# AdrianPerezHerrero/HDP-GPC

Measured on AMD Instinct MI355X. Metric: GP log-lik evals/sec (NxK batch, T-point segments), higher is better.
Workload: dtype f64; 1 GPU; BASELINE configs[1]: synthetic 2048 segments x 8 clusters, T=128, fp64, irregular segment grids (per-pair Gram + Cholesky + score); segments=2048, segments_per_gpu=2048, clusters=8, T=128

## Files before the change

### hdpgpc_amd/csrc/hgp_factor.hip

```cpp
#include <mutex>

#include "hgp_internal.hpp"
#include "tile_f64.hpp"

using namespace hgp;

namespace {

template <int NB>
__global__ __launch_bounds__(64 * WAVES) void k_wave_potrf(PotrfArgs a) {
  __shared__ __attribute__((aligned(16))) double scr_all[WAVES * DIAG_SCR];
  const int wave = threadIdx.x >> 6, lane = threadIdx.x & 63;
  const int g = lane >> 4, c = lane & 15;
  const int m = blockIdx.x * WAVES + wave;
  if (m >= a.b) return;
  double* scr = scr_all + wave * DIAG_SCR;
  double* A = a.A + (size_t)m * a.T * a.T;
  const int T = a.T;
  d4 U[NB * (NB + 1) / 2];
  d4 R[NB];
  load_sym_upper<NB>(U, A, T, T, lane, scr);
  if (a.add != 0.0) add_diag<NB>(U, a.add, T, lane);
  if (a.jitter_rel != 0.0) {
    double dm = diag_abs_mean<NB>(U, T, lane);
    add_diag<NB>(U, a.jitter_rel * fmax(dm, F64_EPS), T, lane);
  }
  PivotAcc pa;
  pa.init();
  wave_factor<NB, 0>(U, R, scr, nullptr, nullptr, lane, pa, A, T, T);
#pragma unroll
  for (int I = 0; I < NB; ++I)
#pragma unroll
    for (int J = I + 1; J < NB; ++J) {
      const int ln = launder(lane);
#pragma unroll
      for (int r = 0; r < 4; ++r) {
        int i = 16 * I + (ln >> 4) + 4 * r, j = 16 * J + (ln & 15);
        if (i < T && j < T) A[(size_t)i * T + j] = 0.0;
      }
    }
  if (lane == 0) {
    if (a.info) a.info[m] = pa.info;
    if (a.logdet) a.logdet[m] = pa.logdet();
  }
}

template <int NB>
__global__ __launch_bounds__(64 * WAVES) void k_wave_inv(PotrfArgs a) {
  __shared__ __attribute__((aligned(16))) double scr_all[WAVES * DIAG_SCR];
  const int wave = threadIdx.x >> 6, lane = threadIdx.x & 63;
  const int g = lane >> 4, c = lane & 15;
  const int w = blockIdx.x * WAVES + wave;
  const int m = w / NB, Jc = w % NB;
  const int T = a.T;
  if (m >= a.b || 16 * Jc >= T) return;
  double* scr = scr_all + wave * DIAG_SCR;
  const double* A = a.A + (size_t)m * T * T;
  d4 U[NB * (NB + 1) / 2];
  d4 R[NB];
  if (a.symmetric) load_upper_only<NB>(U, A, T, T, lane);
  else if constexpr (NB <= 6) load_sym_upper_burst<NB>(U, A, T, T, lane, scr);
  else load_sym_upper<NB>(U, A, T, T, lane, scr);
  {
    double sh = a.add;
    if (a.jitter_rel != 0.0) sh += a.jitter_rel * fmax(diag_abs_mean<NB>(U, T, lane, a.add), F64_EPS);
    if (sh != 0.0) add_diag<NB>(U, sh, T, lane);
  }
#pragma unroll
  for (int K = 0; K < NB; ++K)
#pragma unroll
    for (int r = 0; r < 4; ++r) R[K][r] = (K == Jc && g + 4 * r == c) ? 1.0 : 0.0;
  PivotAcc pa;
  pa.init();
  wave_factor<NB, 1>(U, R, scr, nullptr, nullptr, lane, pa, nullptr, 0, T);
  double* Z = a.Linv + (size_t)m * T * T;
#pragma unroll
  for (int K = 0; K < NB; ++K)
#pragma unroll
    for (int r = 0; r < 4; ++r) {
      const int i = 16 * K + g + 4 * r, j = 16 * Jc + c;
      if (i < T && j < T) Z[(size_t)i * T + j] = (K >= Jc) ? R[K][r] : 0.0;
    }
  if (a.inv_info && Jc == 0 && lane == 0 && a.info) a.info[m] = pa.info;
}

template <int NB>
void launch_wave_inv(const PotrfArgs& a, hipStream_t st) {
  const int waves = a.b * NB;
  hipLaunchKernelGGL(k_wave_inv<NB>, dim3((waves + WAVES - 1) / WAVES), dim3(64 * WAVES), 0, st, a);
}

struct ScoreArgs {
  const double* Y;
  int ldy;
  const double* mean;
  long mean_stride;
  const double* Sigma;
  long sigma_stride;
  int T;
  int ld_sigma;
  const int32_t* item_mat;
  const int32_t* item_mean;
  const double* item_add;
  const int32_t* item_off;
  const int32_t* item_cnt;
  int n_items;
  const int32_t* seg_ids;
  double jitter_rel;
  double* out_quad;
  double* out_logdet;
  int32_t* out_info;
};

template <int NB>
__global__ __launch_bounds__(64 * WAVES) void k_wave_score(ScoreArgs a) {
  __shared__ __attribute__((aligned(16))) double scr_all[WAVES * DIAG_SCR];
  __shared__ __attribute__((aligned(16))) double w_all[WAVES * NB * 256];
  const int wave = threadIdx.x >> 6, lane = threadIdx.x & 63;
  const int g = lane >> 4, c = lane & 15;
  const int it = blockIdx.x * WAVES + wave;
  if (it >= a.n_items) return;
  double* scr = scr_all + wave * DIAG_SCR;
  const int T = a.T;
  const int mat = a.item_mat[it];
  const double* S = a.Sigma + (size_t)mat * a.sigma_stride;
  const double* mu = a.mean ? a.mean + (size_t)(a.item_mean ? a.item_mean[it] : mat) * a.mean_stride : nullptr;
  d4 U[NB * (NB + 1) / 2];
  d4 R[NB];
  double* Wl = w_all + wave * NB * 256;
  load_sym_upper<NB>(U, S, a.ld_sigma, T, lane, scr);
  const double add = a.item_add ? a.item_add[it] : 0.0;
  if (add != 0.0) add_diag<NB>(U, add, T, lane);
  if (a.jitter_rel != 0.0) {
    double dm = diag_abs_mean<NB>(U, T, lane);
    add_diag<NB>(U, a.jitter_rel * fmax(dm, F64_EPS), T, lane);
  }
  const int off = a.item_off[it], cnt = a.item_cnt[it];
  PivotAcc pa;
  pa.init();
  double ld = 0.0;
  for (int base = 0; base < cnt; base += 16) {
    const int j = base + c;
    const bool live = j < cnt;
    const int seg = live ? (a.seg_ids ? a.seg_ids[off + j] : off + j) : 0;
    const double* yr = a.Y + (size_t)seg * a.ldy;
#pragma unroll
    for (int K = 0; K < NB; ++K)
#pragma unroll
      for (int r = 0; r < 4; ++r) {
        int i = 16 * K + g + 4 * r;
        double v = 0.0;
        if (live && i < T) v = yr[i] - (mu ? mu[i] : 0.0);
        R[K][r] = v;
      }
    if (base == 0) {
      wave_factor<NB, 1>(U, R, scr, cnt > 16 ? Wl : nullptr, nullptr, lane, pa, nullptr, 0, T);
      ld = pa.logdet();
    } else {
      wave_fwd_solve<NB>(U, Wl, R, lane);
    }
    double q = wave_colnorm2<NB>(R);
    if (live && g == 0) {
      a.out_quad[seg] = q;
      if (a.out_logdet) a.out_logdet[seg] = ld;
      if (a.out_info) a.out_info[seg] = pa.info;
    }
  }
}

struct EachArgs {
  const double* Y;
  int ldy;
  const double* mean;
  long mean_stride;
  const double* Sigma;
  long sigma_stride;
  int T, n;
  const int32_t* seg_mat;
  const int32_t* seg_mean;
  const double* seg_add;
  double jitter_rel;
  double* out_quad;
  double* out_logdet;
  int32_t* out_info;
  int symmetric;
};

template <int NB, bool SYM>
__global__ __launch_bounds__(64 * WAVES, (NB <= 6) ? 2 : 1) void k_wave_score1(EachArgs a) {
  __shared__ __attribute__((aligned(16))) double scr_all[WAVES * DIAG_SCR];
  __shared__ __attribute__((aligned(16))) double dv_all[WAVES * 16 * NB];
  const int wave = threadIdx.x >> 6, lane = threadIdx.x & 63;
  const int seg = blockIdx.x * WAVES + wave;
  if (seg >= a.n) return;
  double* scr = scr_all + wave * DIAG_SCR;
  double* dv = dv_all + wave * 16 * NB;
  const int T = a.T;
  const int mat = a.seg_mat[seg];
  const double* S = a.Sigma + (size_t)mat * a.sigma_stride;
  const double* mu = a.mean ? a.mean + (size_t)(a.seg_mean ? a.seg_mean[seg] : mat) * a.mean_stride : nullptr;
  const double* yr = a.Y + (size_t)seg * a.ldy;
  for (int i = lane; i < 16 * NB; i += 64) dv[i] = (i < T) ? yr[i] - (mu ? mu[i] : 0.0) : 0.0;
  d4 U[NB * (NB + 1) / 2];
  d4 Rnone[NB];
  if constexpr (SYM) load_upper_only<NB>(U, S, T, T, lane);
  else load_sym_upper<NB>(U, S, T, T, lane, scr);
  {
    double sh = a.seg_add ? a.seg_add[seg] : 0.0;
    if (a.jitter_rel != 0.0) sh += a.jitter_rel * fmax(diag_abs_mean<NB>(U, T, lane, sh), F64_EPS);
    if (sh != 0.0) add_diag<NB>(U, sh, T, lane);
  }
  __builtin_amdgcn_wave_barrier();
  PivotAcc pa;
  pa.init();
  const double q = wave_factor<NB, 2, (NB < 8)>(U, Rnone, scr, nullptr, dv, lane, pa, nullptr, 0, T);
  if (lane == 0) {
    a.out_quad[seg] = q;
    if (a.out_logdet) a.out_logdet[seg] = pa.logdet();
    if (a.out_info) a.out_info[seg] = pa.info;
  }
}

template <int NB>
__global__ __launch_bounds__(64 * WAVES) void k_coop_score(ScoreArgs a) {
  using C = Coop<NB>;
  extern __shared__ __attribute__((aligned(16))) double smem[];
  double* rowbuf = smem;
  double* Rbuf = rowbuf + NB * 256;
  double* Wbuf = Rbuf + NB * 256;
  double* scr = Wbuf + 256;
  double* red = scr + DIAG_SCR;
  int* redi = reinterpret_cast<int*>(red + 8);
  const int wave = __builtin_amdgcn_readfirstlane(threadIdx.x >> 6), lane = threadIdx.x & 63;
  const int g = lane >> 4, c = lane & 15;
  const int it = blockIdx.x;
  const int T = a.T;
  const int mat = a.item_mat[it];
  const double* S = a.Sigma + (size_t)mat * a.sigma_stride;
  const double* mu = a.mean ? a.mean + (size_t)(a.item_mean ? a.item_mean[it] : mat) * a.mean_stride : nullptr;
  const double add = a.item_add ? a.item_add[it] : 0.0;
  const int off = a.item_off[it], cnt = a.item_cnt[it];
  d4 U[C::NT];
  for (int base = 0; base < cnt; base += 16) {
    coop_load_sym_upper<NB>(U, S, a.ld_sigma, T, wave, lane, rowbuf + wave * DIAG_SCR);
    __syncthreads();
    {
      double sh = add;
      if (a.jitter_rel != 0.0) {
        const double dm = coop_diag_abs_mean<NB>(U, T, wave, lane, add, red);
        sh += a.jitter_rel * fmax(dm, F64_EPS);
      }
      if (sh != 0.0) coop_add_diag<NB>(U, sh, T, wave, lane);
    }
    const int j = base + c;
    const bool live = j < cnt;
    const int seg = live ? (a.seg_ids ? a.seg_ids[off + j] : off + j) : 0;
    const double* yr = a.Y + (size_t)seg * a.ldy;
    for (int K = wave; K < NB; K += WAVES) {
      d4 v;
#pragma unroll
      for (int r = 0; r < 4; ++r) {
        const int i = 16 * K + g + 4 * r;
        v[r] = (live && i < T) ? yr[i] - (mu ? mu[i] : 0.0) : 0.0;
      }
      lds_tile_store(Rbuf, K, lane, v);
    }
    __syncthreads();
    PivotAcc pa;
    pa.init();
    coop_factor<NB, true>(U, rowbuf, Rbuf, Wbuf, scr, wave, lane, pa, nullptr, 0, T);
    int info;
    const double ld = coop_logdet_info(pa, wave, lane, red, redi, info);
    double q = 0.0;
    for (int K = wave; K < NB; K += WAVES) {
      const d4 z = lds_tile_load(Rbuf, K, lane);
#pragma unroll
      for (int r = 0; r < 4; ++r) q = fma(z[r], z[r], q);
    }
    q = xrow_sum(q);
    if (g == 0) Wbuf[wave * 16 + c] = q;
    __syncthreads();
    if (wave == 0 && g == 0 && live) {
      a.out_quad[seg] = Wbuf[c] + Wbuf[16 + c] + Wbuf[32 + c] + Wbuf[48 + c];
      if (a.out_logdet) a.out_logdet[seg] = ld;
      if (a.out_info) a.out_info[seg] = info;
    }
    __syncthreads();
  }
}

template <int NB>
__global__ __launch_bounds__(64 * WAVES) void k_coop_potrf(PotrfArgs a) {
  using C = Coop<NB>;
  extern __shared__ __attribute__((aligned(16))) double smem[];
  double* rowbuf = smem;
  double* Rbuf = rowbuf + NB * 256;
  double* Wbuf = Rbuf + NB * 256;
  double* scr = Wbuf + 256;
  double* red = scr + DIAG_SCR;
  int* redi = reinterpret_cast<int*>(red + 8);
  const int wave = __builtin_amdgcn_readfirstlane(threadIdx.x >> 6), lane = threadIdx.x & 63;
  const int m = blockIdx.x;
  const int T = a.T;
  double* A = (a.Aout ? a.Aout : a.A) + (size_t)m * T * T;
  d4 U[C::NT];
  coop_load_sym_upper<NB>(U, a.A + (size_t)m * T * T, T, T, wave, lane, rowbuf + wave * DIAG_SCR);
  __syncthreads();
  {
    double sh = a.add;
    if (a.jitter_rel != 0.0) {
      const double dm = coop_diag_abs_mean<NB>(U, T, wave, lane, a.add, red);
      sh += a.jitter_rel * fmax(dm, F64_EPS);
    }
    if (sh != 0.0) coop_add_diag<NB>(U, sh, T, wave, lane);
  }
  __syncthreads();
  PivotAcc pa;
  pa.init();
  coop_factor<NB, false>(U, rowbuf, Rbuf, Wbuf, scr, wave, lane, pa, A, T, T, nullptr,
                         a.Linv ? a.Linv + (size_t)m * T * T : nullptr, T);
  int info;
  const double ld = coop_logdet_info(pa, wave, lane, red, redi, info);
  if (threadIdx.x == 0) {
    if (a.info) a.info[m] = info;
    if (a.logdet) a.logdet[m] = ld;
  }
  for (int idx = threadIdx.x; idx < T * T; idx += 64 * WAVES) {
    const int i = idx / T, j = idx % T;
    if ((j >> 4) > (i >> 4)) A[idx] = 0.0;
  }
}

template <int NB>
__global__ __launch_bounds__(64 * WAVES) void k_trtri(const double* __restrict__ Lall, double* __restrict__ Zall, int T, int b,
                                                      const int32_t* __restrict__ info) {
  const int wave = threadIdx.x >> 6, lane = threadIdx.x & 63;
  const int g = lane >> 4, c = lane & 15;
  const int w = blockIdx.x * WAVES + wave;
  const int m = w / NB, Kc = w % NB;
  if (m >= b || 16 * Kc >= T) return;
  const double* L = Lall + (size_t)m * T * T;
  double* Z = Zall + (size_t)m * T * T;
  const int nb = (T + 15) >> 4;
  d4 Zc[NB];
#pragma unroll
  for (int I = 0; I < NB; ++I) {
    if (I == Kc) {
#pragma unroll
      for (int r = 0; r < 4; ++r) {
        const int row = 16 * I + g + 4 * r, col = 16 * I + c;
        Zc[I][r] = (row < T && col < T) ? Z[(size_t)row * T + col] : ((row == col) ? 1.0 : 0.0);
      }
    } else {
      Zc[I] = (d4){0.0, 0.0, 0.0, 0.0};
    }
  }
#pragma unroll
  for (int I = 1; I < NB; ++I) {
    if (I > Kc && I < nb) {
      d4 acc0 = (d4){0.0, 0.0, 0.0, 0.0}, acc1 = (d4){0.0, 0.0, 0.0, 0.0};
#pragma unroll
      for (int j = 0; j < I; ++j) {
        if (j >= Kc) {
          double av[4];
#pragma unroll
          for (int s = 0; s < 4; ++s) {
            const int row = 16 * I + c, col = 16 * j + 4 * s + g;
            av[s] = (row < T) ? L[(size_t)row * T + col] : 0.0;
          }
          if (j & 1) {
#pragma unroll
            for (int s = 0; s < 4; ++s) acc1 = mfma(av[s], Zc[j][s], acc1);
          } else {
#pragma unroll
            for (int s = 0; s < 4; ++s) acc0 = mfma(av[s], Zc[j][s], acc0);
          }
        }
      }
#pragma unroll
      for (int r = 0; r < 4; ++r) acc0[r] += acc1[r];
      double wv[4];
#pragma unroll
      for (int s = 0; s < 4; ++s) {
        const int row = 16 * I + c, col = 16 * I + 4 * s + g;
        wv[s] = (row < T && col < T) ? Z[(size_t)row * T + col] : ((row == col) ? 1.0 : 0.0);
      }
      d4 z = (d4){0.0, 0.0, 0.0, 0.0};
#pragma unroll
      for (int s = 0; s < 4; ++s) z = mfma_sub(wv[s], acc0[s], z);
      Zc[I] = z;
    }
  }
  const bool bad = info && info[m] != 0;
#pragma unroll
  for (int I = 0; I < NB; ++I) {
#pragma unroll
    for (int r = 0; r < 4; ++r) {
      const int row = 16 * I + g + 4 * r, col = 16 * Kc + c;
      if (row < T && col < T && I != Kc) Z[(size_t)row * T + col] = bad ? __builtin_nan("") : ((I > Kc) ? Zc[I][r] : 0.0);
    }
  }
}

template <int NB>
__global__ __launch_bounds__(64 * WAVES) void k_coop_inv(PotrfArgs a) {
  using C = Coop<NB>;
  extern __shared__ __attribute__((aligned(16))) double smem[];
  double* rowbuf = smem;
  double* Rbuf = rowbuf + NB * 256;
  double* Wbuf = Rbuf + NB * 256;
  double* scr = Wbuf + 256;
  double* red = scr + DIAG_SCR;
  const int wave = __builtin_amdgcn_readfirstlane(threadIdx.x >> 6), lane = threadIdx.x & 63;
  const int g = lane >> 4, c = lane & 15;
  const int m = blockIdx.x, Jc = blockIdx.y;
  const int T = a.T;
  if (16 * Jc >= T) return;
  const double* A = a.A + (size_t)m * T * T;
  d4 U[C::NT];
  coop_load_sym_upper<NB>(U, A, T, T, wave, lane, rowbuf + wave * DIAG_SCR);
  __syncthreads();
  {
    double sh = a.add;
    if (a.jitter_rel != 0.0) {
      const double dm = coop_diag_abs_mean<NB>(U, T, wave, lane, a.add, red);
      sh += a.jitter_rel * fmax(dm, F64_EPS);
    }
    if (sh != 0.0) coop_add_diag<NB>(U, sh, T, wave, lane);
  }
  for (int K = wave; K < NB; K += WAVES) {
    d4 v;
#pragma unroll
    for (int r = 0; r < 4; ++r) v[r] = (K == Jc && g + 4 * r == c) ? 1.0 : 0.0;
    lds_tile_store(Rbuf, K, lane, v);
  }
  __syncthreads();
  PivotAcc pa;
  pa.init();
  coop_factor<NB, true>(U, rowbuf, Rbuf, Wbuf, scr, wave, lane, pa, nullptr, 0, T);
  double* Z = a.Linv + (size_t)m * T * T;
  for (int K = wave; K < NB; K += WAVES) {
    const d4 z = lds_tile_load(Rbuf, K, lane);
#pragma unroll
    for (int r = 0; r < 4; ++r) {
      const int i = 16 * K + g + 4 * r, j = 16 * Jc + c;
      if (i < T && j < T) Z[(size_t)i * T + j] = (K >= Jc) ? z[r] : 0.0;
    }
  }
  if (a.inv_info && Jc == 0) {
    int info;
    (void)coop_logdet_info(pa, wave, lane, red, reinterpret_cast<int*>(red + 8), info);
    if (threadIdx.x == 0 && a.info) a.info[m] = info;
  }
}

template <int NB>
int launch_coop_score(const ScoreArgs& a, hipStream_t st) {
  const size_t lds = sizeof(double) * Coop<NB>::LDS_DOUBLES;
  if (int rc_ = hgp_internal_ensure_dynamic_lds(reinterpret_cast<const void*>(&k_coop_score<NB>), lds)) return rc_;
  hipLaunchKernelGGL(k_coop_score<NB>, dim3(a.n_items), dim3(64 * WAVES), lds, st, a);
  return launch_status();
}

template <int NB>
int launch_coop_potrf(const PotrfArgs& a, hipStream_t st) {
  const size_t lds = sizeof(double) * Coop<NB>::LDS_DOUBLES;
  if (int rc_ = hgp_internal_ensure_dynamic_lds(reinterpret_cast<const void*>(&k_coop_potrf<NB>), lds)) return rc_;
  if (int rc_ = hgp_internal_ensure_dynamic_lds(reinterpret_cast<const void*>(&k_coop_inv<NB>), lds)) return rc_;
  hipLaunchKernelGGL(k_coop_potrf<NB>, dim3(a.b), dim3(64 * WAVES), lds, st, a);
  if (a.Linv) {
    const int waves = a.b * NB;
    hipLaunchKernelGGL(k_trtri<NB>, dim3((waves + WAVES - 1) / WAVES), dim3(64 * WAVES), 0, st, a.Aout ? a.Aout : a.A, a.Linv, a.T, a.b,
                       a.info);
  }
  return launch_status();
}

template <int NB>
int launch_coop_inv_only(const PotrfArgs& a, hipStream_t st) {
  const size_t lds = sizeof(double) * Coop<NB>::LDS_DOUBLES;
  if (int rc_ = hgp_internal_ensure_dynamic_lds(reinterpret_cast<const void*>(&k_coop_inv<NB>), lds)) return rc_;
  hipLaunchKernelGGL(k_coop_inv<NB>, dim3(a.b, NB), dim3(64 * WAVES), lds, st, a);
  return launch_status();
}

}

int hgp_internal_ensure_dynamic_lds(const void* fn, size_t bytes) {
  static std::mutex mu;
  static std::vector<std::pair<const void*, int>> done;
  int dv = 0;
  if (hipGetDevice(&dv) != hipSuccess) return launch_status();
  std::lock_guard<std::mutex> lk(mu);
  for (const auto& d : done)
    if (d.first == fn && d.second == dv) return 0;
  const hipError_t e = hipFuncSetAttribute(fn, hipFuncAttributeMaxDynamicSharedMemorySize, (int)bytes);
  if (e != hipSuccess) return 1000 + (int)e;
  done.emplace_back(fn, dv);
  return 0;
}

int hgp_internal_chol_inverse(const PotrfArgs& a, int NB, hipStream_t st) {
  if (NB > 8) return dispatch_nb_coop(16 * NB, [&](auto nb) { return launch_coop_potrf<decltype(nb)::value>(a, st); });
  if (NB == 8) return launch_coop_inv_only<8>(a, st);
  dispatch_nb_wave(16 * NB, [&](auto nb) { launch_wave_inv<decltype(nb)::value>(a, st); });
  return launch_status();
}

extern "C" {

int hgp_potrf_batched_f64(double* A, int T, int b, double jitter_rel, double add_diag, double* Linv, double* logdet,
                          int32_t* info, void* stream) {
  if (b == 0) return 0;
  if (!A || T <= 0 || b < 0) return -1;
  if (T > HGP_MAX_T_COOP) return -2;
  PotrfArgs a{A, T, b, jitter_rel, add_diag, Linv, logdet, info};
  hipStream_t st = (hipStream_t)stream;
  if (T > HGP_MAX_T_WAVE) return dispatch_nb_coop(T, [&](auto nb) { return launch_coop_potrf<decltype(nb)::value>(a, st); });
  dispatch_nb_wave(T, [&](auto nb) {
    constexpr int NB = decltype(nb)::value;
    if (Linv) launch_wave_inv<NB>(a, st);
    hipLaunchKernelGGL(k_wave_potrf<NB>, dim3((b + WAVES - 1) / WAVES), dim3(64 * WAVES), 0, st, a);
  });
  return launch_status();
}

int hgp_score_groups_f64(const double* Y, int ldy, const double* mean, long mean_stride, const double* Sigma,
                         long sigma_stride, int T, const int32_t* item_mat, const int32_t* item_mean,
                         const double* item_add, const int32_t* item_off, const int32_t* item_cnt, int n_items,
                         const int32_t* seg_ids, double jitter_rel, double* out_quad, double* out_logdet,
                         int32_t* out_info, void* stream) {
  if (n_items == 0) return 0;
  if (!Y || !Sigma || !item_mat || !item_off || !item_cnt || !out_quad || T <= 0 || ldy < T || n_items < 0) return -1;
  if (T > HGP_MAX_T_COOP) return -2;
  ScoreArgs a{Y, ldy, mean, mean_stride, Sigma, sigma_stride, T, T, item_mat, item_mean, item_add, item_off, item_cnt, n_items,
              seg_ids, jitter_rel, out_quad, out_logdet, out_info};
  hipStream_t st = (hipStream_t)stream;
  if (T > HGP_MAX_T_WAVE) return dispatch_nb_coop(T, [&](auto nb) { return launch_coop_score<decltype(nb)::value>(a, st); });
  dispatch_nb_wave(T, [&](auto nb) {
    hipLaunchKernelGGL(k_wave_score<decltype(nb)::value>, dim3((n_items + WAVES - 1) / WAVES), dim3(64 * WAVES), 0, st, a);
  });
  return launch_status();
}

int hgp_score_each_f64(const double* Y, int ldy, const double* mean, long mean_stride, const double* Sigma,
                       long sigma_stride, int T, const int32_t* seg_mat, const int32_t* seg_mean, const double* seg_add,
                       int n, double jitter_rel, int symmetric, double* out_quad, double* out_logdet, int32_t* out_info,
                       void* stream) {
  if (n == 0) return 0;
  if (!Y || !Sigma || !seg_mat || !out_quad || T <= 0 || ldy < T || n < 0) return -1;
  if (T > HGP_MAX_T_WAVE) return -2;
  EachArgs a{Y, ldy, mean, mean_stride, Sigma, sigma_stride, T, n, seg_mat, seg_mean, seg_add, jitter_rel, out_quad, out_logdet,
             out_info, symmetric};
  hipStream_t st = (hipStream_t)stream;
  dispatch_nb_wave(T, [&](auto nb) {
    dispatch_bool(symmetric != 0, [&](auto sym) {
      hipLaunchKernelGGL((k_wave_score1<decltype(nb)::value, decltype(sym)::value>), dim3((n + WAVES - 1) / WAVES), dim3(64 * WAVES), 0, st, a);
    });
  });
  return launch_status();
}

int hgp_chol_inverse_batched_f64(const double* A, int T, int b, double jitter_rel, double add_diag, double* Linv,
                                 int32_t* info, void* stream) {
  if (b == 0) return 0;
  if (!A || !Linv || T <= 0 || b < 0) return -1;
  if (T > HGP_MAX_T_COOP) return -2;
  PotrfArgs a{const_cast<double*>(A), T, b, jitter_rel, add_diag, Linv, nullptr, info};
  a.inv_info = 1;
  hipStream_t st = (hipStream_t)stream;
  if (T > HGP_MAX_T_WAVE) return dispatch_nb_coop(T, [&](auto nb) { return launch_coop_inv_only<decltype(nb)::value>(a, st); });
  dispatch_nb_wave(T, [&](auto nb) { launch_wave_inv<decltype(nb)::value>(a, st); });
  return launch_status();
}

int hgp_chol_inverse_ws_f64(const double* A, int T, int b, double jitter_rel, double add_diag, double* Linv, double* work,
                            int32_t* info, void* stream) {
  if (b == 0) return 0;
  if (!A || !Linv || T <= 0 || b < 0) return -1;
  if (T > HGP_MAX_T_COOP) return -2;
  const int nb = T <= 192 ? 12 : 16;
  if (T <= HGP_MAX_T_WAVE || !work || (long)b * nb <= 512) return hgp_chol_inverse_batched_f64(A, T, b, jitter_rel, add_diag, Linv, info, stream);
  PotrfArgs a{const_cast<double*>(A), T, b, jitter_rel, add_diag, Linv, nullptr, info};
  a.Aout = work;
  return dispatch_nb_coop(T, [&](auto nbc) { return launch_coop_potrf<decltype(nbc)::value>(a, (hipStream_t)stream); });
}

}
```

### hdpgpc_amd/csrc/hgp_gemm.hip

```cpp
#include <algorithm>

#include "hgp_internal.hpp"
#include "tile_f64.hpp"

using namespace hgp;

namespace {

template <int TRIP>
__global__ __launch_bounds__(64 * WAVES) void k_gemm(GemmArgs a) {
  const int wave = threadIdx.x >> 6, lane = threadIdx.x & 63;
  const int g = lane >> 4, c = lane & 15;
  const int ntn = (a.N + 15) / 16, ntm = (a.M + 15) / 16;
  const int tile = blockIdx.x * WAVES + wave;
  if (tile >= ntm * ntn) return;
  const int ti = tile / ntn, tj = tile % ntn;
  const int by = (int)blockIdx.y + a.boff;
  const int b1 = by / a.nb2, b2 = by % a.nb2;
  const double* A = a.A + (size_t)b1 * a.sA + (size_t)b2 * a.sA2;
  const double* B = a.B + (size_t)b1 * a.sB + (size_t)b2 * a.sB2;
  double* C = a.C + (size_t)b1 * a.sC + (size_t)b2 * a.sC2;
  d4 acc = (d4){0.0, 0.0, 0.0, 0.0};
  const int row = 16 * ti + c, col = 16 * tj + c;
  int nk = (a.Kd + 3) / 4;
  if (a.triA && !a.tA) nk = min(nk, 4 * (ti + 1));
  for (int k0 = 0; k0 < nk; k0 += TRIP) {
    double av[TRIP], bv[TRIP];
#pragma unroll
    for (int u = 0; u < TRIP; ++u) {
      const int k = 4 * (k0 + u) + g;
      av[u] = 0.0;
      bv[u] = 0.0;
      if (k < a.Kd) {
        if (row < a.M) av[u] = a.tA ? A[(size_t)k * a.lda + row] : A[(size_t)row * a.lda + k];
        if (col < a.N) bv[u] = a.tB ? B[(size_t)col * a.ldb + k] : B[(size_t)k * a.ldb + col];
      }
    }
#pragma unroll
    for (int u = 0; u < TRIP; ++u) acc = mfma(av[u], bv[u], acc);
  }
#pragma unroll
  for (int r = 0; r < 4; ++r) {
    const int i = 16 * ti + g + 4 * r;
    if (i < a.M && col < a.N) {
      double v = a.alpha * acc[r];
      if (a.beta != 0.0)
        v += a.beta * (a.D ? a.D[(size_t)b1 * a.sD + (size_t)i * a.ldd + col] : C[(size_t)i * a.ldc + col]);
      C[(size_t)i * a.ldc + col] = v;
    }
  }
}

__global__ __launch_bounds__(64 * WAVES) void k_gemm22(GemmArgs a) {
  const int wave = threadIdx.x >> 6, lane = threadIdx.x & 63;
  const int g = lane >> 4, c = lane & 15;
  const int ntn = a.N / 32, ntm = a.M / 32;
  const int tile = blockIdx.x * WAVES + wave;
  if (tile >= ntm * ntn) return;
  const int ti = tile / ntn, tj = tile % ntn;
  const int by = (int)blockIdx.y + a.boff;
  const int b1 = by / a.nb2, b2 = by % a.nb2;
  const double* A = a.A + (size_t)b1 * a.sA + (size_t)b2 * a.sA2 + (size_t)(32 * ti + c) * a.lda + g;
  const double* B = a.B + (size_t)b1 * a.sB + (size_t)b2 * a.sB2 + (size_t)g * a.ldb + 32 * tj + c;
  double* C = a.C + (size_t)b1 * a.sC + (size_t)b2 * a.sC2;
  d4 acc[2][2];
#pragma unroll
  for (int i = 0; i < 2; ++i)
#pragma unroll
    for (int j = 0; j < 2; ++j) acc[i][j] = (d4){0.0, 0.0, 0.0, 0.0};
  int nk = a.Kd / 4;
  if (a.triA) nk = min(nk, 8 * (ti + 1));
  constexpr int TR = 8;
  for (int k0 = 0; k0 < nk; k0 += TR) {
    double av[TR][2], bv[TR][2];
#pragma unroll
    for (int u = 0; u < TR; ++u) {
      const size_t k = 4 * (size_t)(k0 + u);
      av[u][0] = A[k];
      av[u][1] = A[k + 16 * (size_t)a.lda];
      bv[u][0] = B[k * a.ldb];
      bv[u][1] = B[k * a.ldb + 16];
    }
#pragma unroll
    for (int u = 0; u < TR; ++u) {
#pragma unroll
      for (int i = 0; i < 2; ++i)
#pragma unroll
        for (int j = 0; j < 2; ++j) acc[i][j] = mfma(av[u][i], bv[u][j], acc[i][j]);
    }
  }
#pragma unroll
  for (int i = 0; i < 2; ++i)
#pragma unroll
    for (int j = 0; j < 2; ++j)
#pragma unroll
      for (int r = 0; r < 4; ++r) {
        const int row = 32 * ti + 16 * i + g + 4 * r, col = 32 * tj + 16 * j + c;
        double v = a.alpha * acc[i][j][r];
        if (a.beta != 0.0) v += a.beta * (a.D ? a.D[(size_t)b1 * a.sD + (size_t)row * a.ldd + col] : C[(size_t)row * a.ldc + col]);
        C[(size_t)row * a.ldc + col] = v;
      }
}

__global__ __launch_bounds__(256) void k_dot_batched(const double* __restrict__ X, const double* __restrict__ Y, long sX,
                                                      long sY, long n, double scale, int accumulate, double* out) {
  __shared__ double red[256];
  const double* x = X + (size_t)blockIdx.x * sX;
  const double* y = Y + (size_t)blockIdx.x * sY;
  double s = 0.0;
  for (long i = threadIdx.x; i < n; i += 256) s = fma(x[i], y[i], s);
  red[threadIdx.x] = s;
  __syncthreads();
  for (int o = 128; o > 0; o >>= 1) {
    if (threadIdx.x < o) red[threadIdx.x] += red[threadIdx.x + o];
    __syncthreads();
  }
  if (threadIdx.x == 0) out[blockIdx.x] = (accumulate ? out[blockIdx.x] : 0.0) + scale * red[0];
}

__global__ __launch_bounds__(256) void k_colnorm_diag(const double* __restrict__ Z, const double* __restrict__ S, long sS, int T,
                                                       double scale, int accumulate, double* out) {
  __shared__ double red[256];
  const double* z = Z + (size_t)blockIdx.x * T * T;
  const double* sd = S + (size_t)blockIdx.x * sS;
  double s = 0.0;
  for (long i = threadIdx.x; i < (long)T * T; i += 256) {
    const int r = (int)(i / T), cidx = (int)(i % T);
    if (cidx <= r) {
      const double v = z[i];
      s = fma(v * v, sd[(size_t)cidx * T + cidx], s);
    }
  }
  red[threadIdx.x] = s;
  __syncthreads();
  for (int o = 128; o > 0; o >>= 1) {
    if (threadIdx.x < o) red[threadIdx.x] += red[threadIdx.x + o];
    __syncthreads();
  }
  if (threadIdx.x == 0) out[blockIdx.x] = (accumulate ? out[blockIdx.x] : 0.0) + scale * red[0];
}

__global__ void k_sub_batched(const double* __restrict__ A, const double* __restrict__ B, long sA, long sB, long n,
                              double* __restrict__ C, int b) {
  const size_t i = (size_t)blockIdx.x * blockDim.x + threadIdx.x;
  if (i >= (size_t)n) return;
  for (int m = blockIdx.y; m < b; m += gridDim.y) C[(size_t)m * n + i] = A[(size_t)m * sA + i] - B[(size_t)m * sB + i];
}

}

int hgp_internal_gemm(const GemmArgs& a0, int batch, hipStream_t st) {
  const int nt = ((a0.M + 15) / 16) * ((a0.N + 15) / 16);
  for (int b0 = 0; b0 < batch; b0 += 65535) {
    GemmArgs a = a0;
    a.boff = b0;
    const int nb = std::min(65535, batch - b0);
    if (!a.tA && !a.tB && a.M % 32 == 0 && a.N % 32 == 0 && a.Kd % 32 == 0 && a.Kd > 128 &&
        (long)(a.M / 32) * (a.N / 32) * nb >= 2048) {
      const int nt2 = (a.M / 32) * (a.N / 32);
      hipLaunchKernelGGL(k_gemm22, dim3((nt2 + WAVES - 1) / WAVES, nb), dim3(64 * WAVES), 0, st, a);
      continue;
    }
    if (a.Kd <= 96 && a.Kd > 32)
      hipLaunchKernelGGL(k_gemm<24>, dim3((nt + WAVES - 1) / WAVES, nb), dim3(64 * WAVES), 0, st, a);
    else if (a.Kd <= 128 && a.Kd > 96)
      hipLaunchKernelGGL(k_gemm<32>, dim3((nt + WAVES - 1) / WAVES, nb), dim3(64 * WAVES), 0, st, a);
    else
      hipLaunchKernelGGL(k_gemm<8>, dim3((nt + WAVES - 1) / WAVES, nb), dim3(64 * WAVES), 0, st, a);
  }
  return launch_status();
}

void hgp_internal_dot_batched(const double* X, const double* Y, long sX, long sY, long n, double scale, int accumulate, double* out, int b, hipStream_t st) {
  hipLaunchKernelGGL(k_dot_batched, dim3(b), dim3(256), 0, st, X, Y, sX, sY, n, scale, accumulate, out);
}

void hgp_internal_colnorm_diag(const double* Z, const double* S, long sS, int T, double scale, int accumulate, double* out, int b, hipStream_t st) {
  hipLaunchKernelGGL(k_colnorm_diag, dim3(b), dim3(256), 0, st, Z, S, sS, T, scale, accumulate, out);
}

void hgp_internal_sub_batched(const double* A, const double* B, long sA, long sB, long n, double* C, int b, hipStream_t st) {
  hipLaunchKernelGGL(k_sub_batched, dim3((unsigned)((n + 255) / 256), std::min(b, 65535)), dim3(256), 0, st, A, B, sA, sB, n, C, b);
}

extern "C" {

int hgp_gemm_batched_f64(int transA, int transB, int M, int N, int Kd, double alpha, const double* A, int lda, long strideA,
                         const double* B, int ldb, long strideB, double beta, double* C, int ldc, long strideC, int batch,
                         void* stream) {
  if (!A || !B || !C || M <= 0 || N <= 0 || Kd <= 0 || batch < 0) return -1;
  if (batch == 0) return 0;
  GemmArgs g{A, B, C, M, N, Kd, lda, ldb, ldc, strideA, strideB, strideC, alpha, beta, transA, transB};
  return hgp_internal_gemm(g, batch, (hipStream_t)stream);
}

int hgp_gemm_add_batched_f64(int transA, int transB, int M, int N, int Kd, double alpha, const double* A, int lda, long strideA,
                             const double* B, int ldb, long strideB, double beta, const double* D, int ldd, long strideD,
                             double* C, int ldc, long strideC, int batch, void* stream) {
  if (!A || !B || !C || !D || M <= 0 || N <= 0 || Kd <= 0 || batch < 0) return -1;
  if (batch == 0) return 0;
  GemmArgs g{A, B, C, M, N, Kd, lda, ldb, ldc, strideA, strideB, strideC, alpha, beta, transA, transB};
  g.D = D;
  g.ldd = ldd;
  g.sD = strideD;
  return hgp_internal_gemm(g, batch, (hipStream_t)stream);
}

}
```

### hdpgpc_amd/csrc/hgp_internal.hpp

```cpp
#pragma once
#include <hip/hip_runtime.h>
#include <stdint.h>
#include <stdlib.h>

#include <type_traits>
#include <vector>

#include "../../include/hdpgpc_hip.h"

constexpr int WAVES = 4;

static inline int launch_status() {
  hipError_t e = hipGetLastError();
  return e == hipSuccess ? 0 : 1000 + (int)e;
}

static inline int nb_for(int n) {
  int nb = (n + 15) / 16;
  nb = (nb + 1) & ~1;
  return nb < 2 ? 2 : nb;
}

template <class F> static inline auto dispatch_nb_wave(int T, F&& f) {
  switch (nb_for(T)) {
    case 2: return f(std::integral_constant<int, 2>{});
    case 4: return f(std::integral_constant<int, 4>{});
    case 6: return f(std::integral_constant<int, 6>{});
    default: return f(std::integral_constant<int, 8>{});
  }
}
template <class F> static inline auto dispatch_nb_coop(int T, F&& f) {
  return T <= 192 ? f(std::integral_constant<int, 12>{}) : f(std::integral_constant<int, 16>{});
}
template <class F> static inline auto dispatch_nb(int NB, F&& f) {
  return NB <= 8 ? dispatch_nb_wave(16 * NB, f) : dispatch_nb_coop(16 * NB, f);
}
template <class F> static inline auto dispatch_bool(bool on, F&& f) {
  return on ? f(std::true_type{}) : f(std::false_type{});
}

static inline bool env_on(const char* name) {
  const char* v = getenv(name);
  return v && v[0] && v[0] != '0';
}

constexpr double PAIRS_CUT = 55.45177444479562;
constexpr int PAIRS_FB_CAP = 65536;

static inline int acc_grid_for(int nb) { return nb > 8 ? 256 : 512; }

struct hgp_pairs_plan {
  int T, K, TP, NB;
  std::vector<double> theta;
  std::vector<int32_t> perm;
  std::vector<int> grp_beg, grp_end;
  std::vector<double> grp_ell;
  double *d_theta, *d_scal, *d_A, *d_S, *d_Z, *d_Kinv, *d_P, *d_Q, *d_Mp, *d_ap, *d_xb;
  int32_t* d_perm;
  bool coop = false;
  double* d_escr = nullptr;
  int32_t* d_eflags = nullptr;
  int nscr = 0;
  long escr_stride = 0;
  double acc_tol = 1e-9;
  double* d_Lop = nullptr;
  double* d_LTop = nullptr;
  double* d_Dop = nullptr;
  double* d_Sop = nullptr;
  double* d_mu = nullptr;
  int32_t* d_acc_list = nullptr;
  double* d_sscr = nullptr;
  int32_t* d_fb = nullptr;
  int score_out = 0;
};

struct PotrfArgs {
  double* A;
  int T, b;
  double jitter_rel, add;
  double* Linv;
  double* logdet;
  int32_t* info;
  int inv_info = 0;
  int symmetric = 0;
  double* Aout = nullptr;
};
int hgp_internal_chol_inverse(const PotrfArgs& a, int NB, hipStream_t st);
int hgp_internal_ensure_dynamic_lds(const void* fn, size_t bytes);

struct GemmArgs {
  const double* A;
  const double* B;
  double* C;
  int M, N, Kd, lda, ldb, ldc;
  long sA, sB, sC;
  double alpha, beta;
  int tA, tB;
  int nb2 = 1;
  long sA2 = 0, sB2 = 0, sC2 = 0;
  const double* D = nullptr;
  int ldd = 0;
  long sD = 0;
  int boff = 0;
  int triA = 0;
};
int hgp_internal_gemm(const GemmArgs& a, int batch, hipStream_t st);
void hgp_internal_dot_batched(const double* X, const double* Y, long sX, long sY, long n, double scale, int accumulate, double* out, int b, hipStream_t st);
void hgp_internal_colnorm_diag(const double* Z, const double* S, long sS, int T, double scale, int accumulate, double* out, int b, hipStream_t st);
void hgp_internal_sub_batched(const double* A, const double* B, long sA, long sB, long n, double* C, int b, hipStream_t st);

int hgp_internal_acc_prep(hgp_pairs_plan* p, const double* mean, hipStream_t st);
int hgp_internal_pairs_acc(const hgp_pairs_plan* p, const double* x, const double* y, int N, int Ts, const double* first_noise,
                           const int32_t* sel, double* out_quad, double* out_logdet, int32_t* out_info, hipStream_t st);
size_t hgp_internal_acc_bytes(int TP, int K, size_t* sizes );

int hgp_internal_lat_coop(const double* f_cur, const double* f_prev, const double* A, const double* Gamma, const double* P, int T, int b,
                          double* out, int32_t* info, double* ws, hipStream_t st);
int hgp_internal_mniw_coop(const double* M, const double* Sigma, const double* m_mean, const double* scale, long prior_stride, int T, int b,
                           double* out, int32_t* info, double* ws, hipStream_t st);

struct PairsArgs {
  const double* x;
  const double* y;
  int N, Ts;
  const double* xb;
  int T;
  const double* Mp;
  const double* ap;
  const double* scal;
  const int32_t* perm;
  int kbeg, kend;
  double ell;
  const double* first_noise;
  const int32_t* sel;
#ifdef HGP_STAMPS
  unsigned long long* stamps;
#endif
  int K;
  double* out_quad;
  double* out_logdet;
  int32_t* out_info;
  double* escr;
  int32_t* eflags;
  int nscr;
  long escr_stride;
  int flags;
  double score_add;
  int score_on;
  int32_t* fb;
};

#ifdef HGP_STAMPS
extern unsigned long long* hgp_internal_stamp_dev;
#endif
int hgp_internal_pairs_fast(const PairsArgs& a, int NB, bool coop, hipStream_t st);
```

### hdpgpc_amd/csrc/hgp_pairs_acc.hip

```cpp
#include <hip/hip_runtime.h>
#include <math.h>
#include <stdint.h>

#include "hgp_internal.hpp"
#include "tile_f64.hpp"

using namespace hgp;

namespace {

__host__ __device__ constexpr int ntl(int NB) { return NB * (NB - 1) / 2; }
__host__ __device__ constexpr int tl(int K, int Kp) { return K * (K - 1) / 2 + Kp; }

__global__ void k_acc_flags(double* scal, int K, double tol, int32_t* acc_list) {
  if (threadIdx.x != 0 || blockIdx.x != 0) return;
  int n = 0;
  for (int k = 0; k < K; ++k) {
    const double ck = scal[8 * k] * scal[8 * k + 6];
    const double bound = F64_EPS * ck * ck;
    const bool flag = (tol == 0.0) || (tol > 0.0 && !(bound <= tol));
    scal[8 * k + 7] = flag ? 1.0 : 0.0;
    if (flag) acc_list[1 + n++] = k;
  }
  acc_list[0] = n;
}

template <int NB>
__global__ __launch_bounds__(64) void k_acc_factor(double* A, int TP, const double* scal, int32_t* info) {
  __shared__ __attribute__((aligned(16))) double scr[DIAG_SCR];
  const int k = blockIdx.x, lane = threadIdx.x;
  if (scal[8 * k + 7] == 0.0) return;
  double* Ak = A + (size_t)k * TP * TP;
  d4 U[NB * (NB + 1) / 2];
  d4 R[NB];
  load_upper_only<NB>(U, Ak, TP, TP, lane);
  PivotAcc pa;
  pa.init();
  wave_factor<NB, 0>(U, R, scr, nullptr, nullptr, lane, pa, Ak, TP, TP);
  if (lane == 0 && info && pa.info != 0) info[k] = pa.info;
}

struct AccPrepArgs {
  const double* L;
  const double* S;
  const double* mean;
  const double* scal;
  int T, TP, NB;
  double* Lop;
  double* LTop;
  double* Dop;
  double* Sop;
  double* mu;
};

__global__ __launch_bounds__(256) void k_acc_prep(AccPrepArgs a) {
  const int k = blockIdx.x;
  if (a.scal[8 * k + 7] == 0.0) return;
  const int lane = threadIdx.x & 63, g = lane >> 4, c = lane & 15;
  const int wv = blockIdx.y * 4 + (threadIdx.x >> 6), nwv = gridDim.y * 4;
  const int NB = a.NB, TP = a.TP;
  const double* L = a.L + (size_t)k * TP * TP;
  const double* S = a.S + (size_t)k * TP * TP;
  const int nl = ntl(NB);
  double* Lop = a.Lop + (size_t)k * nl * 256;
  double* LTop = a.LTop + (size_t)k * nl * 256;
  double* Dop = a.Dop + (size_t)k * 4 * NB * 256;
  double* Sop = a.Sop + (size_t)k * NB * NB * 256;
  if (blockIdx.y == 0)
    for (int i = threadIdx.x; i < TP; i += 256) a.mu[(size_t)k * TP + i] = (i < a.T) ? a.mean[(size_t)k * a.T + i] : 0.0;
  const int items = nl + NB + NB * NB;
  for (int it = wv; it < items; it += nwv) {
    if (it < nl) {
      int Kb = 1;
      while (tl(Kb + 1, 0) <= it) ++Kb;
      const int Kp = it - tl(Kb, 0);
      d4 lo, lt;
#pragma unroll
      for (int s = 0; s < 4; ++s) {
        lo[s] = L[(size_t)(16 * Kb + c) * TP + 16 * Kp + 4 * s + g];
        lt[s] = L[(size_t)(16 * Kb + 4 * s + g) * TP + 16 * Kp + c];
      }
      *reinterpret_cast<d4*>(Lop + ((size_t)it * 64 + lane) * 4) = lo;
      *reinterpret_cast<d4*>(LTop + ((size_t)it * 64 + lane) * 4) = lt;
    } else if (it < nl + NB) {
      const int Kb = it - nl;
      const double* D = L + (size_t)(16 * Kb) * TP + 16 * Kb;
      d4 a1, a2, a1t, a2t;
#pragma unroll
      for (int r = 0; r < 4; ++r) {
        const double* B = D + (size_t)(4 * r) * TP + 4 * r;
        const double l00 = B[0], l10 = B[TP], l11 = B[TP + 1], l20 = B[2 * TP], l21 = B[2 * TP + 1], l22 = B[2 * TP + 2],
                     l30 = B[3 * (size_t)TP], l31 = B[3 * (size_t)TP + 1], l32 = B[3 * (size_t)TP + 2], l33 = B[3 * (size_t)TP + 3];
        double w[4][4];
#pragma unroll
        for (int i = 0; i < 4; ++i)
#pragma unroll
          for (int j = 0; j < 4; ++j) w[i][j] = 0.0;
        const double r0 = 1.0 / l00, r1 = 1.0 / l11, r2 = 1.0 / l22, r3 = 1.0 / l33;
        w[0][0] = r0;
        w[1][0] = -(l10 * w[0][0]) * r1;
        w[2][0] = -(l20 * w[0][0] + l21 * w[1][0]) * r2;
        w[3][0] = -(l30 * w[0][0] + l31 * w[1][0] + l32 * w[2][0]) * r3;
        w[1][1] = r1;
        w[2][1] = -(l21 * w[1][1]) * r2;
        w[3][1] = -(l31 * w[1][1] + l32 * w[2][1]) * r3;
        w[2][2] = r2;
        w[3][2] = -(l32 * w[2][2]) * r3;
        w[3][3] = r3;
        const int ci = c & 3;
        double wf = 0.0, wt = 0.0;
#pragma unroll
        for (int i = 0; i < 4; ++i)
#pragma unroll
          for (int j = 0; j < 4; ++j) {
            if (i == ci && j == g) wf = w[i][j];
            if (i == g && j == ci) wt = w[i][j];
          }
        const bool mine = (c >> 2) == r;
        a1[r] = mine ? wf : 0.0;
        a1t[r] = mine ? wt : 0.0;
        a2[r] = (c >= 4 * r + 4) ? D[(size_t)c * TP + 4 * r + g] : 0.0;
        a2t[r] = (c < 4 * r) ? D[(size_t)(4 * r + g) * TP + c] : 0.0;
      }
      *reinterpret_cast<d4*>(Dop + ((size_t)(0 * NB + Kb) * 64 + lane) * 4) = a1;
      *reinterpret_cast<d4*>(Dop + ((size_t)(1 * NB + Kb) * 64 + lane) * 4) = a2;
      *reinterpret_cast<d4*>(Dop + ((size_t)(2 * NB + Kb) * 64 + lane) * 4) = a1t;
      *reinterpret_cast<d4*>(Dop + ((size_t)(3 * NB + Kb) * 64 + lane) * 4) = a2t;
    } else {
      const int t = it - nl - NB, Kb = t / NB, Kp = t % NB;
      d4 so;
#pragma unroll
      for (int s = 0; s < 4; ++s) so[s] = S[(size_t)(16 * Kp + 4 * s + g) * TP + 16 * Kb + c];
      *reinterpret_cast<d4*>(Sop + ((size_t)t * 64 + lane) * 4) = so;
    }
  }
}

struct AccArgs {
  const double* x;
  const double* y;
  int N, Ts;
  const double* xb;
  int T;
  const double* scal;
  const double* mu;
  const double* Lop;
  const double* LTop;
  const double* Dop;
  const double* Sop;
  const int32_t* acc_list;
  const double* first_noise;
  const int32_t* sel;
  int K;
  double* out_quad;
  double* out_logdet;
  int32_t* out_info;
  double* sscr;
  double score_add;
  int score_on;
};

template <int NB>
struct AccLds {
  static constexpr int TP = 16 * NB;
  static constexpr size_t DOUBLES = (size_t)NB * 256  + 256  + 5 * TP  + DIAG_SCR + 32;
  static constexpr size_t BYTES = DOUBLES * sizeof(double) + 16 * sizeof(int);
};

__device__ __forceinline__ d4 ld4(const double* base, unsigned off) { return *reinterpret_cast<const d4*>(base + off); }

template <int NB>
__global__ __launch_bounds__(64 * CoopH<NB>::NW, (NB <= 8) ? 2 : 1) void k_pairs_acc(AccArgs a) {
  using H = CoopH<NB>;
  constexpr int NW = H::NW, TP = 16 * NB;
  extern __shared__ __attribute__((aligned(16))) double smem[];
  double* rowbuf = smem;
  double* Wbuf = rowbuf + NB * 256;
  double* dvec = Wbuf + 256;
  double* xs = dvec + TP;
  double* ys = xs + TP;
  double* xbs = ys + TP;
  double* mus = xbs + TP;
  double* scr = mus + TP;
  double* red = scr + DIAG_SCR;
  int* redi = reinterpret_cast<int*>(red + 32);
  const int tid = threadIdx.x, lane = tid & 63, g = lane >> 4, c = lane & 15;
  const int wave = __builtin_amdgcn_readfirstlane(tid >> 6);
  const int T = a.T, Ts = a.Ts;
  const int nflag = a.acc_list[0];
  if (nflag == 0) return;
  const long npairs = a.sel ? (long)a.N : (long)a.N * nflag;
  double* Ssc = a.sscr + (size_t)blockIdx.x * NB * NB * 256;

  for (long p = blockIdx.x; p < npairs; p += gridDim.x) {
    int n, kc;
    if (a.sel) {
      n = (int)p;
      kc = a.sel[n];
      if (a.scal[8 * kc + 7] == 0.0) continue;
    } else {
      n = (int)(p / nflag);
      kc = a.acc_list[1 + (int)(p % nflag)];
    }
    kc = __builtin_amdgcn_readfirstlane(kc);
    const double* sc = a.scal + 8 * kc;
    const double cc = sc[0], ell = sc[1], noise = sc[2];
    const bool iso = sc[3] != 0.0;
    const size_t oidx = a.sel ? (size_t)n : (size_t)n * a.K + kc;
    const double fn = a.first_noise ? a.first_noise[oidx] : 0.0;
    __syncthreads();
    for (int i = tid; i < TP; i += 64 * NW) {
      xs[i] = (i < Ts) ? a.x[(size_t)n * Ts + i] / ell : 1e150 * (double)(1 + i);
      ys[i] = (i < Ts) ? a.y[(size_t)n * Ts + i] : 0.0;
      xbs[i] = (i < T) ? a.xb[i] / ell : -1e150 * (double)(1 + i);
      mus[i] = a.mu[(size_t)kc * TP + i];
    }
    __syncthreads();
    const double* Lop = a.Lop + (size_t)kc * ntl(NB) * 256;
    const double* LTop = a.LTop + (size_t)kc * ntl(NB) * 256;
    const double* Dop = a.Dop + (size_t)kc * 4 * NB * 256;
    const double* Sop = a.Sop + (size_t)kc * NB * NB * 256;
    double* Sl = Ssc;

    double dsq = 0.0;
#pragma unroll
    for (int q = 0; q < 2; ++q) {
      const int J = (q == 0) ? wave : NB - 1 - wave;
      d4 X[NB];
#pragma unroll
      for (int K = 0; K < NB; ++K) {
        const unsigned l4 = (unsigned)launder(lane) * 4u;
        {
          const int ln = launder(lane);
          const double xj = xs[16 * J + (ln & 15)];
#pragma unroll
          for (int r = 0; r < 4; ++r) {
            const double u = xbs[16 * K + 4 * r + (ln >> 4)] - xj;
            X[K][r] = cc * exp(-0.5 * (u * u));
          }
        }
#pragma unroll
        for (int Kp = 0; Kp < K; ++Kp) {
          const d4 lo = ld4(Lop + tl(K, Kp) * 256, l4);
#pragma unroll
          for (int s = 0; s < 4; ++s) X[K] = mfma_sub(lo[s], X[Kp][s], X[K]);
        }
        const d4 a1 = ld4(Dop + (0 * NB + K) * 256, l4), a2 = ld4(Dop + (1 * NB + K) * 256, l4);
#pragma unroll
        for (int r = 0; r < 4; ++r) {
          d4 t = X[K];
          t[r] = 0.0;
          t = mfma(a1[r], X[K][r], t);
          X[K] = (r < 3) ? mfma_sub(a2[r], t[r], t) : t;
        }
      }
#pragma unroll
      for (int K = NB - 1; K >= 0; --K) {
        const unsigned l4 = (unsigned)launder(lane) * 4u;
#pragma unroll
        for (int Kp = NB - 1; Kp > K; --Kp) {
          const d4 lt = ld4(LTop + tl(Kp, K) * 256, l4);
#pragma unroll
          for (int s = 0; s < 4; ++s) X[K] = mfma_sub(lt[s], X[Kp][s], X[K]);
        }
        const d4 a1 = ld4(Dop + (2 * NB + K) * 256, l4), a2 = ld4(Dop + (3 * NB + K) * 256, l4);
#pragma unroll
        for (int r = 3; r >= 0; --r) {
          d4 t = X[K];
          t[r] = 0.0;
          t = mfma(a1[r], X[K][r], t);
          X[K] = (r > 0) ? mfma_sub(a2[r], t[r], t) : t;
        }
      }
      double pj = 0.0;
#pragma unroll
      for (int K = 0; K < NB; ++K) {
        const int ln = launder(lane);
        const unsigned l4 = (unsigned)ln * 4u;
#pragma unroll
        for (int r = 0; r < 4; ++r) pj = fma(X[K][r], mus[16 * K + 4 * r + (ln >> 4)], pj);
        *reinterpret_cast<d4*>(Sl + (K * NB + J) * 256 + l4) = X[K];
      }
      pj = xrow_sum(pj);
      if (g == 0) {
        const int j = 16 * J + c;
        const double d = ys[j] - pj;
        dvec[j] = d;
        dsq = fma(d, d, dsq);
      }
    }
    __syncthreads();

    if (iso) {
      dsq = wave_sum(dsq);
      if (lane == 0) red[wave] = dsq;
      __syncthreads();
      if (tid == 0) {
        const double v = sc[4] + fn;
        const double v2 = v + 1e-8 * fmax(fabs(v), F64_EPS);
        double tot_ = 0.0;
        for (int w_ = 0; w_ < NW; ++w_) tot_ += red[w_];
        a.out_quad[oidx] = a.score_on ? fma(-0.5, tot_ / v2, a.score_add) : (tot_ / v2);
        if (a.out_logdet) a.out_logdet[oidx] = (double)Ts * log(v2);
        if (a.out_info) a.out_info[oidx] = (v2 > 0.0) ? 0 : 1;
      }
      continue;
    }

    d4 U[H::NT];
#pragma unroll
    for (int q = 0; q < 2; ++q) {
      const int J = (q == 0) ? wave : NB - 1 - wave;
      const double xj = xs[16 * J + c];
#pragma unroll
      for (int I = 0; I < (q == 0 ? NW : NB); ++I) {
        const int ln = launder(lane);
        d4 kt = (d4){0.0, 0.0, 0.0, 0.0};
        if (I <= J) {
#pragma unroll
          for (int r = 0; r < 4; ++r) {
            const double u = xs[16 * I + (ln >> 4) + 4 * r] - xs[16 * J + (ln & 15)];
            kt[r] = cc * exp(-0.5 * (u * u));
          }
          if (I == J) {
#pragma unroll
            for (int r = 0; r < 4; ++r)
              if ((ln >> 4) + 4 * r == (ln & 15)) kt[r] = (16 * I + (ln & 15) < Ts) ? cc + noise : 1.0;
          }
          U[q == 0 ? H::slotA(I) : H::slotB(I)] = kt;
        }
      }
#pragma nounroll
      for (int K = 0; K < NB; ++K) {
        const unsigned l4 = (unsigned)launder(lane) * 4u;
        d4 Q;
#pragma unroll
        for (int r = 0; r < 4; ++r) {
          const double u = xbs[16 * K + 4 * r + g] - xj;
          Q[r] = -(cc * exp(-0.5 * (u * u)));
        }
#pragma unroll
        for (int Kp = 0; Kp < NB; ++Kp) {
          const d4 so = ld4(Sop + (K * NB + Kp) * 256, l4);
          const d4 sb = ld4(Sl + (Kp * NB + J) * 256, l4);
#pragma unroll
          for (int s = 0; s < 4; ++s) Q = mfma(so[s], sb[s], Q);
        }
#pragma unroll
        for (int I = 0; I < (q == 0 ? NW : NB); ++I) {
          if (I <= J) {
            const d4 sa = ld4(Sl + (K * NB + I) * 256, l4);
#pragma unroll
            for (int s = 0; s < 4; ++s)
              U[q == 0 ? H::slotA(I) : H::slotB(I)] = mfma(sa[s], Q[s], U[q == 0 ? H::slotA(I) : H::slotB(I)]);
          }
        }
      }
    }

    {
      const double sh = 1e-6 + fn;
      const double dm = cooph_diag_abs_mean<NB>(U, Ts, wave, lane, sh, red);
      cooph_add_diag<NB>(U, sh + 1e-8 * fmax(dm, F64_EPS), Ts, wave, lane);
    }
    PivotAcc pa;
    pa.init();
    double zq = cooph_factor<NB>(U, rowbuf, Wbuf, scr, wave, lane, pa, Ts, dvec);
    int info;
    const double ld = cooph_logdet_info<NB>(pa, wave, lane, red, redi, info);
    zq = wave_sum(zq);
    if (lane == 0) red[8 + wave] = zq;
    __syncthreads();
    if (tid == 0) {
      double tot_ = 0.0;
      for (int w_ = 0; w_ < NW; ++w_) tot_ += red[8 + w_];
      a.out_quad[oidx] = a.score_on ? fma(-0.5, tot_, a.score_add) : (tot_);
      if (a.out_logdet) a.out_logdet[oidx] = ld;
      if (a.out_info) a.out_info[oidx] = info;
    }
  }
}

template <int NB>
int launch_pairs_acc(const AccArgs& a, hipStream_t st) {
  const size_t lds = AccLds<NB>::BYTES;
  hipLaunchKernelGGL(k_pairs_acc<NB>, dim3(acc_grid_for(NB)), dim3(64 * CoopH<NB>::NW), lds, st, a);
  return launch_status();
}

}

size_t hgp_internal_acc_bytes(int TP, int K, size_t* sizes) {
  const int NB = TP / 16;
  size_t s[6];
  s[0] = (size_t)K * ntl(NB) * 256 * sizeof(double);
  s[1] = s[0];
  s[2] = (size_t)K * 4 * NB * 256 * sizeof(double);
  s[3] = (size_t)K * NB * NB * 256 * sizeof(double);
  s[4] = (size_t)K * TP * sizeof(double);
  s[5] = (size_t)acc_grid_for(NB) * NB * NB * 256 * sizeof(double);
  size_t tot = 0;
  for (int i = 0; i < 6; ++i) {
    if (sizes) sizes[i] = s[i];
    tot += (s[i] + 255) & ~(size_t)255;
  }
  return tot;
}

int hgp_internal_acc_prep(hgp_pairs_plan* p, const double* mean, hipStream_t st) {
  const int K = p->K, TP = p->TP, NB = p->NB;
  hipLaunchKernelGGL(k_acc_flags, dim3(1), dim3(64), 0, st, p->d_scal, K, p->acc_tol, p->d_acc_list);
  if (p->acc_tol < 0.0) return launch_status();
  if (NB <= 8)
    dispatch_nb_wave(TP, [&](auto nb) {
      hipLaunchKernelGGL(k_acc_factor<decltype(nb)::value>, dim3(K), dim3(64), 0, st, p->d_A, TP, p->d_scal, (int32_t*)nullptr);
    });
  AccPrepArgs a{p->d_A, p->d_S, mean, p->d_scal, p->T, TP, NB, p->d_Lop, p->d_LTop, p->d_Dop, p->d_Sop, p->d_mu};
  hipLaunchKernelGGL(k_acc_prep, dim3(K, 8), dim3(256), 0, st, a);
  return launch_status();
}

int hgp_internal_pairs_acc(const hgp_pairs_plan* p, const double* x, const double* y, int N, int Ts, const double* first_noise,
                           const int32_t* sel, double* out_quad, double* out_logdet, int32_t* out_info, hipStream_t st) {
  if (p->acc_tol < 0.0) return 0;
  AccArgs a{x, y, N, Ts, p->d_xb, p->T, p->d_scal, p->d_mu, p->d_Lop, p->d_LTop, p->d_Dop, p->d_Sop, p->d_acc_list,
            first_noise, sel, p->K, out_quad, out_logdet, out_info, p->d_sscr, -0.5 * (double)Ts * 1.8378770664093453, p->score_out};
  return dispatch_nb(p->NB, [&](auto nb) { return launch_pairs_acc<decltype(nb)::value>(a, st); });
}
```

### hdpgpc_amd/csrc/hgp_plan.hip

```cpp
#include <algorithm>
#include <new>

#include "hgp_internal.hpp"
#include "tile_f64.hpp"

using namespace hgp;

namespace {

struct PrepArgs {
  const double* xb;
  const double* mean;
  const double* Sigma;
  int T, TP, K;
  const double* theta;
  double* scal;
  double* A;
  double* S;
  double* xb_copy;
};

__global__ __launch_bounds__(256) void k_prep_build(PrepArgs a) {
  __shared__ double red[256];
  __shared__ int redi[256];
  const int k = blockIdx.x, tid = threadIdx.x;
  const int T = a.T, TP = a.TP;
  const double* Sg = a.Sigma + (size_t)k * T * T;
  const double c = a.theta[3 * k], ell = a.theta[3 * k + 1], noise = a.theta[3 * k + 2];
  double s_abs = 0.0, s_sgn = 0.0;
  for (int i = tid; i < T; i += 256) {
    double d = Sg[(size_t)i * T + i];
    s_abs += fabs(d);
    s_sgn += d;
  }
  red[tid] = s_abs;
  __syncthreads();
  for (int o = 128; o > 0; o >>= 1) {
    if (tid < o) red[tid] += red[tid + o];
    __syncthreads();
  }
  const double mean_abs = red[0] / T;
  __syncthreads();
  red[tid] = s_sgn;
  __syncthreads();
  for (int o = 128; o > 0; o >>= 1) {
    if (tid < o) red[tid] += red[tid + o];
    __syncthreads();
  }
  const double mS = red[0] / T;
  int bad = 0;
  for (int i = tid; i < T; i += 256) {
    double d = Sg[(size_t)i * T + i];
    if (!(fabs(d - mS) <= 1e-8 + 1e-5 * fabs(mS))) bad = 1;
  }
  redi[tid] = bad;
  __syncthreads();
  for (int o = 128; o > 0; o >>= 1) {
    if (tid < o) redi[tid] |= redi[tid + o];
    __syncthreads();
  }
  const double jit = 1e-4 * fmax(mean_abs, F64_EPS);
  if (tid == 0 && blockIdx.y == 0) {
    double* sc = a.scal + 8 * k;
    sc[0] = c;
    sc[1] = ell;
    sc[2] = noise;
    sc[3] = redi[0] ? 0.0 : 1.0;
    sc[4] = mS;
    sc[5] = jit;
    sc[6] = 0.0;
  }
  if (k == 0 && blockIdx.y == 0)
    for (int i = tid; i < TP; i += 256) a.xb_copy[i] = (i < T) ? a.xb[i] : 0.0;
  double* Ak = a.A + (size_t)k * TP * TP;
  double* Sk = a.S + (size_t)k * TP * TP;
  for (int idx = blockIdx.y * 256 + tid; idx < TP * TP; idx += gridDim.y * 256) {
    int i = idx / TP, j = idx % TP;
    double av, sv = 0.0;
    if (i < T && j < T) {
      double u = a.xb[i] / ell - a.xb[j] / ell;
      av = c * exp(-0.5 * (u * u));
      if (i == j) av += jit;
      sv = 0.5 * (Sg[(size_t)i * T + j] + Sg[(size_t)j * T + i]);
    } else {
      av = (i == j) ? 1.0 : 0.0;
    }
    Ak[idx] = av;
    Sk[idx] = sv;
  }
}

struct PrepFinalArgs {
  const double* Q;
  const double* Kinv;
  const double* mean;
  double* scal;
  int T, TP;
  double* Mp;
  double* ap;
  int interleave;
  int32_t* fb;
};

__global__ __launch_bounds__(256) void k_prep_final(PrepFinalArgs a) {
  const int k = blockIdx.x, tid = threadIdx.x;
  if (a.fb && k == 0 && blockIdx.y == 0 && tid == 0) {
    a.fb[0] = 0;
    a.fb[1 + PAIRS_FB_CAP] = 0;
  }
  const int T = a.T, TP = a.TP;
  const double c = a.scal[8 * k];
  const double* Q = a.Q + (size_t)k * TP * TP;
  const double* Ki = a.Kinv + (size_t)k * TP * TP;
  double* Mp = a.Mp + (size_t)k * TP * TP;
  __shared__ double tq[32][33], tk[32][33];
  const int NHh = (TP / 16) / 2, nt = TP / 32;
  const int tx = tid & 31, ty = tid >> 5;
  for (int t = blockIdx.y; t < nt * nt; t += gridDim.y) {
    const int bi = t / nt, bj = t % nt;
    __syncthreads();
#pragma unroll
    for (int r = 0; r < 4; ++r) {
      const int y = ty + 8 * r;
      tq[y][tx] = Q[(size_t)(32 * bj + y) * TP + 32 * bi + tx];
      tk[y][tx] = Ki[(size_t)(32 * bj + y) * TP + 32 * bi + tx];
    }
    __syncthreads();
#pragma unroll
    for (int r = 0; r < 4; ++r) {
      const int y = ty + 8 * r;
      const int i = 32 * bi + y, j = 32 * bj + tx;
      double v = 0.0;
      if (i < T && j < T)
        v = (c * c) * (0.5 * (Q[(size_t)i * TP + j] + tq[tx][y]) - 0.5 * (Ki[(size_t)i * TP + j] + tk[tx][y]));
      int jp = j;
      if (a.interleave) {
        const int hh = j / (16 * NHh), tl = (j / 16) % NHh, cc = j % 16;
        const int loc = (tl < 2 * (NHh / 2)) ? 32 * (tl / 2) + 2 * cc + (tl & 1) : 16 * (NHh - 1) + cc;
        jp = 16 * NHh * hh + loc;
      }
      Mp[(size_t)i * TP + jp] = v;
    }
  }
  const double* mu = a.mean + (size_t)k * T;
  __shared__ double red[256];
  double rmax = 0.0;
  for (int i = blockIdx.y * 256 + tid; i < TP; i += gridDim.y * 256) {
    double s = 0.0, rs = 0.0;
    if (i < T) {
#pragma unroll 8
      for (int j = 0; j < T; ++j) {
        const double kij = Ki[(size_t)j * TP + i];
        s = fma(kij, mu[j], s);
        rs += fabs(kij);
      }
    }
    a.ap[(size_t)k * TP + i] = c * s;
    rmax = fmax(rmax, rs);
  }
  red[tid] = rmax;
  __syncthreads();
  for (int o = 128; o > 0; o >>= 1) {
    if (tid < o) red[tid] = fmax(red[tid], red[tid + o]);
    __syncthreads();
  }
  if (tid == 0) atomicMax(reinterpret_cast<unsigned long long*>(a.scal + 8 * k + 6), (unsigned long long)__double_as_longlong(red[0]));
}

static int tp_for(int n) {
  if (n <= HGP_MAX_T_WAVE) return 16 * nb_for(n);
  return n <= 192 ? 192 : 256;
}

size_t plan_layout(hgp_pairs_plan* p, int T, int Ts_max, int K, char* base) {
  const size_t TP = (size_t)tp_for(std::max(T, Ts_max));
  const size_t mat = (size_t)K * TP * TP * sizeof(double);
  p->TP = (int)TP;
  p->NB = p->TP / 16;
  p->coop = p->TP > HGP_MAX_T_WAVE;
  size_t o = 0;
  auto take = [&](auto*& member, size_t bytes) {
    if (base) member = reinterpret_cast<std::remove_reference_t<decltype(member)>>(base + o);
    o += (bytes + 255) & ~(size_t)255;
  };
  take(p->d_theta, (size_t)K * 3 * sizeof(double));
  take(p->d_scal, (size_t)K * 8 * sizeof(double));
  take(p->d_A, mat);
  take(p->d_S, mat);
  take(p->d_Z, mat);
  take(p->d_Kinv, mat);
  take(p->d_P, mat);
  take(p->d_Q, mat);
  take(p->d_Mp, mat);
  take(p->d_ap, (size_t)K * TP * sizeof(double));
  take(p->d_perm, (size_t)K * sizeof(int32_t));
  take(p->d_xb, TP * sizeof(double));
  if (p->coop) {
    const size_t nb = (size_t)p->NB;
    const size_t cap = (nb >= 12) ? 48 : (nb == 8 ? 24 : 16);
    const size_t over = nb * nb > cap ? nb * nb - cap : 0;
    p->nscr = over ? (nb >= 12 ? 512 : 1024) : 0;
    p->escr_stride = (long)(over * 256);
    take(p->d_escr, (size_t)p->nscr * over * 256 * sizeof(double));
    take(p->d_eflags, ((size_t)p->nscr + 1) * sizeof(int32_t));
  }
  size_t sz[6];
  hgp_internal_acc_bytes((int)TP, K, sz);
  take(p->d_Lop, sz[0]);
  take(p->d_LTop, sz[1]);
  take(p->d_Dop, sz[2]);
  take(p->d_Sop, sz[3]);
  take(p->d_mu, sz[4]);
  take(p->d_sscr, sz[5]);
  take(p->d_acc_list, (size_t)(K + 1) * sizeof(int32_t));
  take(p->d_fb, (size_t)(PAIRS_FB_CAP + 2) * sizeof(int32_t));
  return o;
}

}

#ifdef HGP_STAMPS
unsigned long long* hgp_internal_stamp_dev = nullptr;
#endif

extern "C" {

size_t hgp_pairs_plan_device_bytes(int T, int Ts_max, int K) {
  if (T <= 0 || Ts_max <= 0 || K <= 0) return 0;
  hgp_pairs_plan sizing;
  return plan_layout(&sizing, T, Ts_max, K, nullptr);
}

int hgp_pairs_plan_create(hgp_pairs_plan** plan, int T, int Ts_max, int K, const double* theta_host, void* dev_buf,
                          size_t dev_bytes) {
  if (!plan || !theta_host || !dev_buf || T <= 0 || Ts_max <= 0 || K <= 0) return -1;
  if (T > HGP_MAX_T_COOP || Ts_max > HGP_MAX_T_COOP) return -2;
  if (dev_bytes < hgp_pairs_plan_device_bytes(T, Ts_max, K)) return -1;
  for (int k = 0; k < K; ++k)
    if (!(theta_host[3 * k] > 0.0) || !(theta_host[3 * k + 1] > 0.0)) return -1;
  hgp_pairs_plan* p = new (std::nothrow) hgp_pairs_plan();
  if (!p) return -1;
  p->T = T;
  p->K = K;
  p->theta.assign(theta_host, theta_host + 3 * (size_t)K);
  p->perm.resize(K);
  for (int k = 0; k < K; ++k) p->perm[k] = k;
  std::stable_sort(p->perm.begin(), p->perm.end(),
                   [&](int a, int b) { return p->theta[3 * a + 1] < p->theta[3 * b + 1]; });
  for (int i = 0; i < K;) {
    int j = i;
    double ell = p->theta[3 * p->perm[i] + 1];
    while (j < K && p->theta[3 * p->perm[j] + 1] == ell) ++j;
    p->grp_beg.push_back(i);
    p->grp_end.push_back(j);
    p->grp_ell.push_back(ell);
    i = j;
  }
  plan_layout(p, T, Ts_max, K, (char*)dev_buf);
  if (hipMemset(p->d_fb, 0, (size_t)(PAIRS_FB_CAP + 2) * sizeof(int32_t)) != hipSuccess) {
    delete p;
    return 1000 + (int)hipGetLastError();
  }
  if (p->coop && hipMemset(p->d_eflags, 0, (p->nscr + 1) * sizeof(int32_t)) != hipSuccess) {
    delete p;
    return 1000 + (int)hipGetLastError();
  }
  if (hipMemcpy(p->d_theta, p->theta.data(), sizeof(double) * 3 * K, hipMemcpyHostToDevice) != hipSuccess ||
      hipMemcpy(p->d_perm, p->perm.data(), sizeof(int32_t) * K, hipMemcpyHostToDevice) != hipSuccess) {
    delete p;
    return 1000 + (int)hipGetLastError();
  }
  *plan = p;
  return 0;
}

void hgp_pairs_plan_destroy(hgp_pairs_plan* plan) { delete plan; }

const double* hgp_pairs_plan_scalars(const hgp_pairs_plan* plan) { return plan ? plan->d_scal : nullptr; }

int hgp_pairs_plan_update(hgp_pairs_plan* p, const double* x_basis, const double* mean, const double* Sigma,
                          int32_t* info, void* stream) {
  if (!p || !x_basis || !mean || !Sigma) return -1;
  hipStream_t st = (hipStream_t)stream;
  const int K = p->K, T = p->T, TP = p->TP;
  PrepArgs pa{x_basis, mean, Sigma, T, TP, K, p->d_theta, p->d_scal, p->d_A, p->d_S, p->d_xb};
  hipLaunchKernelGGL(k_prep_build, dim3(K, 8), dim3(256), 0, st, pa);
  PotrfArgs fa{p->d_A, TP, K, 0.0, 0.0, p->d_Z, nullptr, info};
  fa.inv_info = 1;
  fa.symmetric = 1;
  if (int rc = hgp_internal_chol_inverse(fa, p->NB, st)) return rc;
  const long sm = (long)TP * TP;
  GemmArgs g1{p->d_Z, p->d_Z, p->d_Kinv, TP, TP, TP, TP, TP, TP, sm, sm, sm, 1.0, 0.0, 1, 0};
  GemmArgs g2{p->d_S, p->d_Kinv, p->d_P, TP, TP, TP, TP, TP, TP, sm, sm, sm, 1.0, 0.0, 0, 0};
  GemmArgs g3{p->d_Kinv, p->d_P, p->d_Q, TP, TP, TP, TP, TP, TP, sm, sm, sm, 1.0, 0.0, 0, 0};
  hgp_internal_gemm(g1, K, st);
  hgp_internal_gemm(g2, K, st);
  hgp_internal_gemm(g3, K, st);
  PrepFinalArgs fin{p->d_Q, p->d_Kinv, mean, p->d_scal, T, TP, p->d_Mp, p->d_ap, p->coop ? 0 : 1, p->d_fb};
  hipLaunchKernelGGL(k_prep_final, dim3(K, 8), dim3(256), 0, st, fin);
  if (p->d_eflags && p->nscr > 0 && hipMemsetAsync(p->d_eflags, 0, (p->nscr + 1) * sizeof(int32_t), st) != hipSuccess) return launch_status();
  int rc = hgp_internal_acc_prep(p, mean, st);
  return rc ? rc : launch_status();
}

int hgp_pairs_plan_set_accuracy(hgp_pairs_plan* p, double tol) {
  if (!p || tol != tol) return -1;
  p->acc_tol = tol;
  return 0;
}

int hgp_pairs_plan_set_score_output(hgp_pairs_plan* p, int on) {
  if (!p) return -1;
  p->score_out = on ? 1 : 0;
  return 0;
}

int hgp_loglik_pairs_f64(const hgp_pairs_plan* p, const double* x, const double* y, int N, int Ts,
                         const double* first_noise, const int32_t* sel, double* out_quad, double* out_logdet,
                         int32_t* out_info, void* stream) {
  if (N == 0) return 0;
  if (!p || !x || !y || !out_quad || N < 0 || Ts <= 0) return -1;
  if (Ts > HGP_MAX_T_COOP) return -2;
  if (Ts > p->TP) return -2;
  hipStream_t st = (hipStream_t)stream;
  int rc = 0;
  if (p->coop && p->d_eflags && p->nscr > 0 &&
      hipMemsetAsync(p->d_eflags, 0, (p->nscr + 1) * sizeof(int32_t), st) != hipSuccess)
    return launch_status();
  for (size_t gi = 0; gi < p->grp_beg.size() && rc == 0; ++gi) {
    PairsArgs a{x, y, N, Ts, p->d_xb, p->T, p->d_Mp, p->d_ap, p->d_scal, p->d_perm, p->grp_beg[gi], p->grp_end[gi],
                p->grp_ell[gi], first_noise, sel,
#ifdef HGP_STAMPS
                hgp_internal_stamp_dev,
#endif
                p->K, out_quad, out_logdet, out_info, p->d_escr, p->d_eflags, p->nscr, p->escr_stride,
                env_on("HGP_PAIRS_GENERIC") ? 1 : 0, -0.5 * (double)Ts * 1.8378770664093453, p->score_out, p->d_fb};
    rc = hgp_internal_pairs_fast(a, p->NB, p->coop, st);
  }
  if (rc == 0) rc = hgp_internal_pairs_acc(p, x, y, N, Ts, first_noise, sel, out_quad, out_logdet, out_info, st);
  return rc;
}

#ifdef HGP_STAMPS
int hgp_debug_stamps(unsigned long long* out8_host) {
  if (!hgp_internal_stamp_dev) {
    if (hipMalloc(&hgp_internal_stamp_dev, 128) != hipSuccess) return 1;
    (void)hipMemset(hgp_internal_stamp_dev, 0, 128);
  }
  if (hipMemcpy(out8_host, hgp_internal_stamp_dev, 128, hipMemcpyDeviceToHost) != hipSuccess) return 1;
  (void)hipMemset(hgp_internal_stamp_dev, 0, 128);
  return 0;
}
#endif

}
```

### hdpgpc_amd/csrc/tile_f64.hpp

```cpp
#pragma once
#include <hip/hip_runtime.h>
#include <stdint.h>

#include <type_traits>

#ifdef HGP_STAMPS
#define HGP_STAMP_DECL unsigned long long hgp_t_, hgp_acc_[12] = {0, 0, 0, 0, 0, 0, 0, 0, 0, 0, 0, 0};
#define HGP_T0() hgp_t_ = __builtin_readcyclecounter()
#define HGP_ACC(i) do { unsigned long long n_ = __builtin_readcyclecounter(); hgp_acc_[i] += n_ - hgp_t_; hgp_t_ = n_; } while (0)
#else
#define HGP_STAMP_DECL
#define HGP_T0()
#define HGP_ACC(i)
#endif

namespace hgp {

typedef double d4 __attribute__((ext_vector_type(4)));
typedef double d2 __attribute__((ext_vector_type(2)));

constexpr int DIAG_LD = 18;
constexpr int DIAG_SCR = 16 * DIAG_LD;
constexpr double F64_EPS = 2.220446049250313e-16;

__host__ __device__ constexpr int tix(int I, int J, int NB) { return I * NB - (I * (I - 1)) / 2 + (J - I); }
#ifdef HGP_RACE_STRESS
__device__ __forceinline__ void hgp_sync_stress() {
  __syncthreads();
  const unsigned w = threadIdx.x >> 6;
  const unsigned h = ((w + 1u) * 2654435761u) ^ (unsigned)(__builtin_readcyclecounter() >> 9);
  const unsigned n = __builtin_amdgcn_readfirstlane(((h >> 3) & 3u) * 4u);
  for (unsigned i = 0; i < n; ++i) __builtin_amdgcn_s_sleep(32);
}
#define __syncthreads() ::hgp::hgp_sync_stress()
#endif

__host__ __device__ constexpr int ntiles(int NB) { return NB * (NB + 1) / 2; }

__device__ __forceinline__ d4 mfma(double a, double b, d4 c) {
  return __builtin_amdgcn_mfma_f64_16x16x4f64(a, b, c, 0, 0, 0);
}
__device__ __forceinline__ d4 mfma_sub(double a, double b, d4 c) {
  return __builtin_amdgcn_mfma_f64_16x16x4f64(a, b, c, 0, 0, 1);
}

__device__ __forceinline__ int launder(int x) {
  asm volatile("" : "+v"(x));
  return x;
}

__device__ __forceinline__ double launder_f64(double x) {
  asm volatile("" : "+v"(x));
  return x;
}

template <int B, int E, class F>
__device__ __forceinline__ void static_for(F&& f) {
  if constexpr (B < E) {
    f(std::integral_constant<int, B>{});
    static_for<B + 1, E>(f);
  }
}

template <int CTRL>
__device__ __forceinline__ double dpp_f64(double v) {
  const int lo = __builtin_amdgcn_mov_dpp(__double2loint(v), CTRL, 0xf, 0xf, false);
  const int hi = __builtin_amdgcn_mov_dpp(__double2hiint(v), CTRL, 0xf, 0xf, false);
  return __hiloint2double(hi, lo);
}
template <bool MAX>
__device__ __forceinline__ double wave_allreduce(double v) {
  auto op = [](double a, double b) { return MAX ? fmax(a, b) : a + b; };
  v = op(v, dpp_f64<0x128>(v));
  v = op(v, dpp_f64<0x124>(v));
  v = op(v, dpp_f64<0x122>(v));
  v = op(v, dpp_f64<0x121>(v));
  unsigned lo = (unsigned)__double2loint(v), hi = (unsigned)__double2hiint(v);
  auto a = __builtin_amdgcn_permlane16_swap(lo, lo, false, false);
  auto b = __builtin_amdgcn_permlane16_swap(hi, hi, false, false);
  v = op(__hiloint2double((int)b[0], (int)a[0]), __hiloint2double((int)b[1], (int)a[1]));
  lo = (unsigned)__double2loint(v);
  hi = (unsigned)__double2hiint(v);
  a = __builtin_amdgcn_permlane32_swap(lo, lo, false, false);
  b = __builtin_amdgcn_permlane32_swap(hi, hi, false, false);
  return op(__hiloint2double((int)b[0], (int)a[0]), __hiloint2double((int)b[1], (int)a[1]));
}

__device__ __forceinline__ double wave_sum(double v) { return wave_allreduce<false>(v); }

__device__ __forceinline__ double xrow_sum(double v) {
  unsigned lo = (unsigned)__double2loint(v), hi = (unsigned)__double2hiint(v);
  auto a = __builtin_amdgcn_permlane16_swap(lo, lo, false, false);
  auto b = __builtin_amdgcn_permlane16_swap(hi, hi, false, false);
  double s = __hiloint2double((int)b[0], (int)a[0]) + __hiloint2double((int)b[1], (int)a[1]);
  lo = (unsigned)__double2loint(s);
  hi = (unsigned)__double2hiint(s);
  a = __builtin_amdgcn_permlane32_swap(lo, lo, false, false);
  b = __builtin_amdgcn_permlane32_swap(hi, hi, false, false);
  return __hiloint2double((int)b[0], (int)a[0]) + __hiloint2double((int)b[1], (int)a[1]);
}

__device__ __forceinline__ double rsqrt_nr(double a) {
  const double y = __builtin_amdgcn_rsq(a);
  const double e = fma(-(0.5 * a * y), y, 0.5);
  return fma(y * e, fma(1.5, e, 1.0), y);
}

__device__ __forceinline__ void exp_neg4(const double (&h)[4], double (&o)[4]) {
  double n[4], r[4], p[4];
#pragma unroll
  for (int i = 0; i < 4; ++i) {
    const double t = -fmin(h[i], 800.0);
    n[i] = __builtin_rint(t * 1.4426950408889634);
    r[i] = fma(n[i], -6.93147180369123816490e-01, t);
  }
#pragma unroll
  for (int i = 0; i < 4; ++i) {
    r[i] = fma(n[i], -1.90821492927058770002e-10, r[i]);
    p[i] = 1.6059043836821613e-10;
  }
  constexpr double ck[13] = {1.0, 1.0, 0.5, 1.6666666666666666e-01, 4.1666666666666664e-02, 8.3333333333333332e-03,
                             1.3888888888888889e-03, 1.9841269841269841e-04, 2.4801587301587302e-05, 2.7557319223985893e-06,
                             2.7557319223985888e-07, 2.5052108385441720e-08, 2.0876756987868100e-09};
#pragma unroll
  for (int k = 12; k >= 0; --k) {
#pragma unroll
    for (int i = 0; i < 4; ++i) p[i] = fma(p[i], r[i], ck[k]);
  }
#pragma unroll
  for (int i = 0; i < 4; ++i) o[i] = __builtin_amdgcn_ldexp(p[i], (int)n[i]);
}

struct PivotAcc {
  double mant;
  int ex;
  int info;
#ifdef HGP_STAMPS
  unsigned long long diag_cycles, cf[5];
  __device__ __forceinline__ void init() { mant = 1.0; ex = 0; info = 0; diag_cycles = 0; for (int i = 0; i < 5; ++i) cf[i] = 0; }
#else
  __device__ __forceinline__ void init() { mant = 1.0; ex = 0; info = 0; }
#endif
  __device__ __forceinline__ void renorm() {
    ex += __builtin_amdgcn_frexp_exp(mant);
    mant = __builtin_amdgcn_frexp_mant(mant);
  }
  __device__ __forceinline__ double logdet() const { return log(mant) + (double)ex * 0.6931471805599453; }
};

__device__ __forceinline__ double lane_bcast(double v, int src) {
  int lo = __builtin_amdgcn_readlane(__double2loint(v), src);
  int hi = __builtin_amdgcn_readlane(__double2hiint(v), src);
  return __hiloint2double(hi, lo);
}

__device__ __forceinline__ double rcp_nr(double a) {
  const double y = __builtin_amdgcn_rcp(a);
  const double e = fma(-a, y, 1.0);
  const double ye = y * e;
  return fma(ye, e, y + ye);
}

__device__ __forceinline__ double row16_prod(double v) {
  v *= dpp_f64<0x128>(v);
  v *= dpp_f64<0x124>(v);
  v *= dpp_f64<0x122>(v);
  v *= dpp_f64<0x121>(v);
  return v;
}
__device__ __forceinline__ int row16_sum_i32(int v) {
  v += __builtin_amdgcn_mov_dpp(v, 0x128, 0xf, 0xf, false);
  v += __builtin_amdgcn_mov_dpp(v, 0x124, 0xf, 0xf, false);
  v += __builtin_amdgcn_mov_dpp(v, 0x122, 0xf, 0xf, false);
  v += __builtin_amdgcn_mov_dpp(v, 0x121, 0xf, 0xf, false);
  return v;
}

template <int G0>
__device__ __forceinline__ double row_to_all(double v) {
  const unsigned lo = (unsigned)__double2loint(v), hi = (unsigned)__double2hiint(v);
  const auto a = __builtin_amdgcn_permlane16_swap(lo, lo, false, false);
  const auto b = __builtin_amdgcn_permlane16_swap(hi, hi, false, false);
  const unsigned lo1 = a[G0 & 1], hi1 = b[G0 & 1];
  const auto a2 = __builtin_amdgcn_permlane32_swap(lo1, lo1, false, false);
  const auto b2 = __builtin_amdgcn_permlane32_swap(hi1, hi1, false, false);
  return __hiloint2double((int)b2[G0 >> 1], (int)a2[G0 >> 1]);
}
__device__ __forceinline__ double row_to_all_bperm(double v, int addr) {
  const int lo = __builtin_amdgcn_ds_bpermute(addr, __double2loint(v));
  const int hi = __builtin_amdgcn_ds_bpermute(addr, __double2hiint(v));
  return __hiloint2double(hi, lo);
}
template <int RS, int RMF>
__device__ __forceinline__ void elim_crit(double (&S)[4], double (&Z)[4], double mrot, double nt, double ntz) {
  asm("s_nop 1\n\t"
      "v_fmac_f64_dpp %0, %2, %3 row_newbcast:%5 row_mask:%6 bank_mask:0xf\n\t"
      "v_fmac_f64_dpp %1, %2, %4 row_newbcast:%5 row_mask:%6 bank_mask:0xf"
      : "+v"(S[RS]), "+v"(Z[RS])
      : "v"(mrot), "v"(nt), "v"(ntz), "n"(4 * RS), "n"(RMF));
}
template <int RS>
__device__ __forceinline__ void elim_rest(double (&S)[4], double (&Z)[4], double mrot, double nt, double ntz) {
#define HGP_FD(dst, mul, lane) "v_fmac_f64_dpp %" #dst ", %6, %" #mul " row_newbcast:" #lane " row_mask:0xf bank_mask:0xf\n\t"
  if constexpr (RS == 0) {
    asm("s_nop 1\n\t" HGP_FD(0, 7, 4) HGP_FD(1, 7, 8) HGP_FD(2, 7, 12) HGP_FD(3, 8, 4) HGP_FD(4, 8, 8) HGP_FD(5, 8, 12)
        : "+v"(S[1]), "+v"(S[2]), "+v"(S[3]), "+v"(Z[1]), "+v"(Z[2]), "+v"(Z[3])
        : "v"(mrot), "v"(nt), "v"(ntz));
  } else if constexpr (RS == 1) {
    asm("s_nop 1\n\t" HGP_FD(1, 7, 8) HGP_FD(2, 7, 12) HGP_FD(4, 8, 8) HGP_FD(5, 8, 12)
        : "+v"(S[1]), "+v"(S[2]), "+v"(S[3]), "+v"(Z[1]), "+v"(Z[2]), "+v"(Z[3])
        : "v"(mrot), "v"(nt), "v"(ntz));
  } else if constexpr (RS == 2) {
    asm("s_nop 1\n\t" HGP_FD(2, 7, 12) HGP_FD(5, 8, 12)
        : "+v"(S[1]), "+v"(S[2]), "+v"(S[3]), "+v"(Z[1]), "+v"(Z[2]), "+v"(Z[3])
        : "v"(mrot), "v"(nt), "v"(ntz));
  }
#undef HGP_FD
}

struct NoBg {
  template <class KC>
  __device__ __forceinline__ void operator()(KC) const {}
};
template <class BG = NoBg>
__device__ __forceinline__ d4 diag16_acc(const d4& X, double* scr, int lane, PivotAcc& pa, int col0,
                                         double* Lout, int ldl, int nvalid, BG&& bg = BG{}) {
  const int g = lane >> 4, c = lane & 15;
#ifdef HGP_STAMPS
  const unsigned long long td0 = __builtin_readcyclecounter();
#endif
  double S[4], Z[4];
  d4 Us;
#pragma unroll
  for (int r = 0; r < 4; ++r) {
    S[r] = X[r];
    Z[r] = (4 * r + g == c) ? 1.0 : 0.0;
    Us[r] = 0.0;
  }
  int pvlo = 0, pvhi = 0;
  const int crot = (c + g) & 15;
  double p = lane_bcast(S[0], 0);
  double sk = row_to_all_bperm(S[0], 4 * c), mrot = row_to_all_bperm(S[0], 4 * crot), zk = row_to_all_bperm(Z[0], 4 * c);
  static_for<0, 15>([&](auto kc) {
    constexpr int k = decltype(kc)::value, r0 = k >> 2, g0 = k & 3;
    constexpr int RS = (g0 == 3) ? r0 + 1 : r0;
    constexpr int RMF = (g0 == 3) ? 0xf : (0xf << (g0 + 1)) & 0xf;
    asm("v_writelane_b32 %0, %1, %2" : "+v"(pvlo) : "s"(__double2loint(p)), "n"(k));
    asm("v_writelane_b32 %0, %1, %2" : "+v"(pvhi) : "s"(__double2hiint(p)), "n"(k));
    const double rp = rcp_nr(p);
    if (Lout != nullptr) Us[r0] = (g == g0) ? sk : Us[r0];
    const double nt = -(sk * rp), ntz = -(zk * rp), mr = mrot;
    elim_crit<RS, RMF>(S, Z, mr, nt, ntz);
    constexpr int k1 = k + 1, g1 = k1 & 3;
    p = lane_bcast(S[RS], 16 * g1 + k1);
    if constexpr (k1 < 15) {
      scr[lane] = S[RS];
      scr[64 + lane] = Z[RS];
      __builtin_amdgcn_wave_barrier();
      sk = scr[16 * g1 + c];
      zk = scr[64 + 16 * g1 + c];
      mrot = scr[16 * g1 + crot];
      __builtin_amdgcn_wave_barrier();
    }
    bg(kc);
    elim_rest<RS>(S, Z, mr, nt, ntz);
  });
  asm("v_writelane_b32 %0, %1, %2" : "+v"(pvlo) : "s"(__double2loint(p)), "n"(15));
  asm("v_writelane_b32 %0, %1, %2" : "+v"(pvhi) : "s"(__double2hiint(p)), "n"(15));
  if (Lout != nullptr) Us[3] = (g == 3) ? S[3] : Us[3];
  const double pv = row_to_all<0>(__hiloint2double(pvhi, pvlo));
  const double rc = rsqrt_nr(pv);
  {
    const unsigned long long bad = __ballot(!(pv > 0.0)) & 0xffffull;
    if (bad != 0 && pa.info == 0) pa.info = col0 + __ffsll((long long)bad);
    pa.mant *= row16_prod(__builtin_amdgcn_frexp_mant(pv));
    pa.ex += row16_sum_i32(__builtin_amdgcn_frexp_exp(pv));
    pa.renorm();
  }
  if (Lout != nullptr) {
#pragma unroll
    for (int r = 0; r < 4; ++r) scr[(4 * r + g) * DIAG_LD + c] = Us[r];
    if (g == 0) scr[c * DIAG_LD + 16] = rc;
    __builtin_amdgcn_wave_barrier();
    if (lane < 16 && lane < nvalid) {
#pragma unroll
      for (int i = 0; i < 16; ++i)
        if (i < nvalid) Lout[(size_t)lane * ldl + i] = (i <= lane) ? scr[i * DIAG_LD + lane] * scr[i * DIAG_LD + 16] : 0.0;
    }
    __builtin_amdgcn_wave_barrier();
  }
#pragma unroll
  for (int r = 0; r < 4; ++r) scr[(4 * r + g) * DIAG_LD + c] = Z[r];
  __builtin_amdgcn_wave_barrier();
  d4 w;
#pragma unroll
  for (int s = 0; s < 4; ++s) w[s] = scr[c * DIAG_LD + 4 * s + g] * rc;
  __builtin_amdgcn_wave_barrier();
#ifdef HGP_STAMPS
  asm volatile("s_waitcnt lgkmcnt(0)" ::: "memory");
  pa.diag_cycles += __builtin_readcyclecounter() - td0;
#endif
  return w;
}

template <int NB, int Kp>
struct Pending {
  static constexpr int M = NB - 1 - Kp, NT = M * (M + 1) / 2 - 1, N = 4 * NT, CH = (N + 14) / 15;
  static constexpr int row(int t) {
    int u = t + 1, I = Kp + 1;
    while (u >= NB - I) { u -= NB - I; ++I; }
    return I;
  }
  static constexpr int col(int t) {
    int u = t + 1, I = Kp + 1;
    while (u >= NB - I) { u -= NB - I; ++I; }
    return I + u;
  }
};
template <int NB, int RHSMODE, bool RHS_DEFER = false>
__device__ __forceinline__ double wave_factor(d4 (&U)[NB * (NB + 1) / 2], d4 (&R)[NB], double* scr, double* Wlds,
                                              double* dvec, int lane_in, PivotAcc& pa, double* Lout, int ldl, int n) {
  constexpr bool RHS = (RHSMODE == 1);
  double zq = 0.0;
  double dp[NB];
#pragma unroll
  for (int K = 0; K < NB; ++K) dp[K] = 0.0;
  static_for<0, NB>([&](auto Kc) {
    constexpr int K = decltype(Kc)::value;
    const int lane = launder(lane_in);
    const int g = lane >> 4, c = lane & 15;
    double* Ld = (Lout != nullptr) ? Lout + (size_t)(16 * K) * ldl + 16 * K : nullptr;
    d4 W;
    if constexpr (K > 0 && K + 1 < NB) {
      using P = Pending<NB, K - 1>;
      W = diag16_acc(U[tix(K, K, NB)], scr, lane, pa, 16 * K, Ld, ldl, n - 16 * K, [&](auto kc) {
        constexpr int k = decltype(kc)::value, q0 = k * P::CH, q1 = (q0 + P::CH < P::N) ? q0 + P::CH : P::N;
        static_for<q0, q1>([&](auto qc) {
          constexpr int q = decltype(qc)::value, s = q / P::NT, t = q % P::NT, I = P::row(t), J = P::col(t);
          U[tix(I, J, NB)] = mfma_sub(U[tix(K - 1, I, NB)][s], U[tix(K - 1, J, NB)][s], U[tix(I, J, NB)]);
        });
      });
    } else {
      W = diag16_acc(U[tix(K, K, NB)], scr, lane, pa, 16 * K, Ld, ldl, n - 16 * K);
    }
    if (Wlds != nullptr) {
#pragma unroll
      for (int s = 0; s < 4; ++s) Wlds[(K * 4 + s) * 64 + lane] = W[s];
    }
    if (RHSMODE == 2) {
      if (RHS_DEFER && K > 0) {
        const double q = xrow_sum(dp[K]);
        if (g == 0) dvec[16 * K + c] -= q;
        __builtin_amdgcn_wave_barrier();
      }
      double p = 0.0;
#pragma unroll
      for (int s = 0; s < 4; ++s) p = fma(W[s], dvec[16 * K + 4 * s + g], p);
      p = xrow_sum(p);
      __builtin_amdgcn_wave_barrier();
      if (g == 0) {
        dvec[16 * K + c] = p;
        zq = fma(p, p, zq);
      }
      __builtin_amdgcn_wave_barrier();
    }
#pragma unroll
    for (int J0 = K + 1; J0 <= NB; J0 += 2) {
      d4 acc0 = (d4){0.0, 0.0, 0.0, 0.0}, acc1 = (d4){0.0, 0.0, 0.0, 0.0};
      const int J1 = J0 + 1;
      const bool has0 = (J0 < NB) || RHS, has1 = (J1 < NB) || (RHS && J1 == NB);
#pragma unroll
      for (int s = 0; s < 4; ++s) {
        if (has0) acc0 = mfma(W[s], (J0 < NB) ? U[tix(K, J0 < NB ? J0 : K, NB)][s] : R[K][s], acc0);
        if (has1) acc1 = mfma(W[s], (J1 < NB) ? U[tix(K, J1 < NB ? J1 : K, NB)][s] : R[K][s], acc1);
      }
      if (J0 < NB) U[tix(K, J0 < NB ? J0 : K, NB)] = acc0;
      else if (RHS) R[K] = acc0;
      if (J1 < NB) U[tix(K, J1 < NB ? J1 : K, NB)] = acc1;
      else if (RHS && J1 == NB) R[K] = acc1;
    }
    if (Lout != nullptr) {
#pragma unroll
      for (int J = K + 1; J < NB; ++J) {
#pragma unroll
        for (int r = 0; r < 4; ++r) {
          int row = 16 * J + c, col = 16 * K + g + 4 * r;
          if (row < n && col < n) Lout[(size_t)row * ldl + col] = U[tix(K, J, NB)][r];
        }
      }
    }
    if (RHSMODE == 2 && K + 1 < NB) {
      double zr[4];
#pragma unroll
      for (int r = 0; r < 4; ++r) zr[r] = dvec[16 * K + g + 4 * r];
      if (RHS_DEFER) {
#pragma unroll
        for (int I = K + 1; I < NB; ++I) {
#pragma unroll
          for (int r = 0; r < 4; ++r) dp[I] = fma(U[tix(K, I, NB)][r], zr[r], dp[I]);
        }
      } else {
#pragma unroll
        for (int I = K + 1; I < NB; ++I) {
          double q = 0.0;
#pragma unroll
          for (int r = 0; r < 4; ++r) q = fma(U[tix(K, I, NB)][r], zr[r], q);
          q = xrow_sum(q);
          if (g == 0) dvec[16 * I + c] -= q;
        }
        __builtin_amdgcn_wave_barrier();
      }
    }
#pragma unroll
    for (int I = K + 1; I < NB; ++I) {
#pragma unroll
      for (int s = 0; s < 4; ++s) {
#pragma unroll
        for (int J = I; J < NB; ++J) {
          if (K + 2 < NB && !(I == K + 1 && J == K + 1)) continue;
          U[tix(I, J, NB)] = mfma_sub(U[tix(K, I, NB)][s], U[tix(K, J, NB)][s], U[tix(I, J, NB)]);
        }
        if (RHS) R[I] = mfma_sub(U[tix(K, I, NB)][s], R[K][s], R[I]);
      }
    }
  });
  return (RHSMODE == 2) ? wave_sum(zq) : 0.0;
}

template <int NB>
__device__ __forceinline__ void wave_fwd_solve(const d4 (&U)[NB * (NB + 1) / 2], const double* Wlds, d4 (&R)[NB],
                                               int lane, int K0 = 0) {
#pragma unroll
  for (int K = 0; K < NB; ++K) {
    if (K < K0) continue;
    d4 t = R[K];
#pragma unroll
    for (int I = 0; I < K; ++I) {
      if (I < K0) continue;
#pragma unroll
      for (int s = 0; s < 4; ++s) t = mfma_sub(U[tix(I, K, NB)][s], R[I][s], t);
    }
    d4 z = (d4){0.0, 0.0, 0.0, 0.0};
#pragma unroll
    for (int s = 0; s < 4; ++s) z = mfma(Wlds[(K * 4 + s) * 64 + lane], t[s], z);
    R[K] = z;
  }
}

template <int NB>
__device__ __forceinline__ double wave_colnorm2(const d4 (&Z)[NB]) {
  double s = 0.0;
#pragma unroll
  for (int K = 0; K < NB; ++K)
#pragma unroll
    for (int r = 0; r < 4; ++r) s = fma(Z[K][r], Z[K][r], s);
  s += __shfl_xor(s, 16, 64);
  s += __shfl_xor(s, 32, 64);
  return s;
}

template <int NB>
__device__ __forceinline__ void load_sym_upper(d4 (&U)[NB * (NB + 1) / 2], const double* __restrict__ A, int ld, int n,
                                               int lane_in, double* scr) {
#pragma unroll
  for (int I = 0; I < NB; ++I) {
    const int lane = launder(lane_in);
    const int g = lane >> 4, c = lane & 15;
    d4 nat[NB], trn[NB];
#pragma unroll
    for (int J = I; J < NB; ++J) {
#pragma unroll
      for (int r = 0; r < 4; ++r) {
        const int i = 16 * I + g + 4 * r, j = 16 * J + c;
        nat[J][r] = (i < n && j < n) ? A[(size_t)i * ld + j] : 0.0;
        const int i2 = 16 * J + g + 4 * r, j2 = 16 * I + c;
        trn[J][r] = (J > I && i2 < n && j2 < n) ? A[(size_t)i2 * ld + j2] : 0.0;
      }
    }
#pragma unroll
    for (int J = I; J < NB; ++J) {
      const d4 src = (J == I) ? nat[I] : trn[J];
#pragma unroll
      for (int r = 0; r < 4; ++r) scr[(g + 4 * r) * DIAG_LD + c] = src[r];
      __builtin_amdgcn_wave_barrier();
      d4 v;
#pragma unroll
      for (int r = 0; r < 4; ++r) {
        const int i = 16 * I + g + 4 * r, j = 16 * J + c;
        const double t = scr[c * DIAG_LD + g + 4 * r];
        double x = 0.5 * (nat[J][r] + t);
        if (!(i < n && j < n)) x = (i == j) ? 1.0 : 0.0;
        v[r] = x;
      }
      __builtin_amdgcn_wave_barrier();
      U[tix(I, J, NB)] = v;
    }
  }
}

template <int NB>
__device__ __forceinline__ void load_sym_upper_burst(d4 (&U)[NB * (NB + 1) / 2], const double* __restrict__ A, int ld, int n,
                                                     int lane_in, double* scr) {
  constexpr int NO = NB > 1 ? NB * (NB - 1) / 2 : 1;
  d4 trn[NO];
  {
    const int lane = launder(lane_in);
    const int g = lane >> 4, c = lane & 15;
#pragma unroll
    for (int I = 0; I < NB; ++I)
#pragma unroll
      for (int J = I; J < NB; ++J)
#pragma unroll
        for (int r = 0; r < 4; ++r) {
          const int i = 16 * I + g + 4 * r, j = 16 * J + c;
          U[tix(I, J, NB)][r] = (i < n && j < n) ? A[(size_t)i * ld + j] : 0.0;
          if (J > I) {
            const int i2 = 16 * J + g + 4 * r, j2 = 16 * I + c;
            trn[tix(I, J, NB) - (I + 1)][r] = (i2 < n && j2 < n) ? A[(size_t)i2 * ld + j2] : 0.0;
          }
        }
  }
#pragma unroll
  for (int I = 0; I < NB; ++I) {
#pragma unroll
    for (int J = I; J < NB; ++J) {
      const int lane = launder(lane_in);
      const int g = lane >> 4, c = lane & 15;
      const d4 nat = U[tix(I, J, NB)];
      const d4 src = (J == I) ? nat : trn[(J == I) ? 0 : tix(I, J, NB) - (I + 1)];
#pragma unroll
      for (int r = 0; r < 4; ++r) scr[(g + 4 * r) * DIAG_LD + c] = src[r];
      __builtin_amdgcn_wave_barrier();
      d4 v;
#pragma unroll
      for (int r = 0; r < 4; ++r) {
        const int i = 16 * I + g + 4 * r, j = 16 * J + c;
        const double t = scr[c * DIAG_LD + g + 4 * r];
        double x = 0.5 * (nat[r] + t);
        if (!(i < n && j < n)) x = (i == j) ? 1.0 : 0.0;
        v[r] = x;
      }
      __builtin_amdgcn_wave_barrier();
      U[tix(I, J, NB)] = v;
    }
  }
}

template <int NB>
__device__ __forceinline__ void load_upper_only(d4 (&U)[NB * (NB + 1) / 2], const double* __restrict__ A, int ld, int n,
                                                int lane_in) {
#pragma unroll
  for (int I = 0; I < NB; ++I) {
#pragma unroll
    for (int J = I; J < NB; ++J) {
      const int lane = launder(lane_in);
      const int g = lane >> 4, c = lane & 15;
      d4 v;
#pragma unroll
      for (int r = 0; r < 4; ++r) {
        int i = 16 * I + g + 4 * r, j = 16 * J + c;
        double x = 0.0;
        if (i < n && j < n) x = A[(size_t)i * ld + j];
        else if (i == j) x = 1.0;
        v[r] = x;
      }
      U[tix(I, J, NB)] = v;
    }
  }
}

template <int NB>
__device__ __forceinline__ void add_diag(d4 (&U)[NB * (NB + 1) / 2], double shift, int n, int lane_in) {
#pragma unroll
  for (int I = 0; I < NB; ++I) {
    const int lane = launder(lane_in);
    const int g = lane >> 4, c = lane & 15;
#pragma unroll
    for (int r = 0; r < 4; ++r) {
      int i = 16 * I + g + 4 * r;
      if (g + 4 * r == c && i < n) U[tix(I, I, NB)][r] += shift;
    }
  }
}

template <int NB>
__device__ __forceinline__ double diag_abs_mean(const d4 (&U)[NB * (NB + 1) / 2], int n, int lane_in, double shift = 0.0) {
  double s = 0.0;
#pragma unroll
  for (int I = 0; I < NB; ++I) {
    const int lane = launder(lane_in);
    const int g = lane >> 4, c = lane & 15;
#pragma unroll
    for (int r = 0; r < 4; ++r) {
      int i = 16 * I + g + 4 * r;
      if (g + 4 * r == c && i < n) s += fabs(U[tix(I, I, NB)][r] + shift);
    }
  }
  return wave_sum(s) / (double)n;
}

template <int NB>
struct Coop {
  static_assert(NB % 4 == 0 && NB <= 16, "cooperative factor: NB in {4,8,12,16}");
  static constexpr int NQ = NB / 4;
  static constexpr int NT = 2 * NQ * (NQ + 1);
  __host__ __device__ static constexpr int loc(int I, int q) { return 2 * q * (q + 1) + I; }
  __host__ __device__ static constexpr int col(int q, int wave) { return 4 * q + ((q & 1) ? 3 - wave : wave); }
  __host__ __device__ static constexpr int owner(int J) { return ((J >> 2) & 1) ? 3 - (J & 3) : (J & 3); }
  static constexpr int LDS_DOUBLES = NB * 256  + NB * 256  + 256  + DIAG_SCR + 16;
};

__device__ __forceinline__ d4 lds_tile_load(const double* buf, int tile, int lane) {
  d4 v;
#pragma unroll
  for (int r = 0; r < 4; ++r) v[r] = buf[(tile * 4 + r) * 64 + lane];
  return v;
}
__device__ __forceinline__ void lds_tile_store(double* buf, int tile, int lane, const d4& v) {
#pragma unroll
  for (int r = 0; r < 4; ++r) buf[(tile * 4 + r) * 64 + lane] = v[r];
}

template <int NB>
__device__ __forceinline__ void coop_load_sym_upper(d4 (&U)[Coop<NB>::NT], const double* __restrict__ A, int ld, int n,
                                                    int wave, int lane_in, double* scr_w) {
#pragma unroll
  for (int q = 0; q < Coop<NB>::NQ; ++q) {
    const int lane = launder(lane_in);
    const int g = lane >> 4, c = lane & 15;
    const int J = Coop<NB>::col(q, wave);
    d4 nat[NB], trn[NB];
#pragma unroll
    for (int I = 0; I < 4 * q + 4; ++I) {
#pragma unroll
      for (int r = 0; r < 4; ++r) {
        const int i = 16 * I + g + 4 * r, j = 16 * J + c;
        nat[I][r] = (I <= J && i < n && j < n) ? A[(size_t)i * ld + j] : 0.0;
        const int i2 = 16 * J + g + 4 * r, j2 = 16 * I + c;
        trn[I][r] = (I < J && i2 < n && j2 < n) ? A[(size_t)i2 * ld + j2] : 0.0;
      }
    }
#pragma unroll
    for (int I = 0; I < 4 * q + 4; ++I) {
      const d4 src = (I == J) ? nat[I] : trn[I];
#pragma unroll
      for (int r = 0; r < 4; ++r) scr_w[(g + 4 * r) * DIAG_LD + c] = src[r];
      __builtin_amdgcn_wave_barrier();
      d4 v = (d4){0.0, 0.0, 0.0, 0.0};
#pragma unroll
      for (int r = 0; r < 4; ++r) {
        const int i = 16 * I + g + 4 * r, j = 16 * J + c;
        const double t = scr_w[c * DIAG_LD + g + 4 * r];
        double x = 0.5 * (nat[I][r] + t);
        if (!(i < n && j < n)) x = (i == j) ? 1.0 : 0.0;
        if (I <= J) v[r] = x;
      }
      __builtin_amdgcn_wave_barrier();
      U[Coop<NB>::loc(I, q)] = v;
    }
  }
}

template <int NB>
__device__ __forceinline__ double coop_diag_abs_mean(const d4 (&U)[Coop<NB>::NT], int n, int wave, int lane_in, double shift,
                                                     double* red) {
  double s = 0.0;
#pragma unroll
  for (int q = 0; q < Coop<NB>::NQ; ++q) {
#pragma unroll
    for (int I = 4 * q; I < 4 * q + 4; ++I) {
      const int lane = launder(lane_in);
      const int g = lane >> 4, c = lane & 15;
      if (I == Coop<NB>::col(q, wave)) {
#pragma unroll
        for (int r = 0; r < 4; ++r) {
          const int i = 16 * I + g + 4 * r;
          if (g + 4 * r == c && i < n) s += fabs(U[Coop<NB>::loc(I, q)][r] + shift);
        }
      }
    }
  }
  s = wave_sum(s);
  if (lane_in == 0) red[wave] = s;
  __syncthreads();
  const double tot = red[0] + red[1] + red[2] + red[3];
  __syncthreads();
  return tot / (double)n;
}

template <int NB>
__device__ __forceinline__ void coop_add_diag(d4 (&U)[Coop<NB>::NT], double shift, int n, int wave, int lane_in) {
#pragma unroll
  for (int q = 0; q < Coop<NB>::NQ; ++q) {
#pragma unroll
    for (int I = 4 * q; I < 4 * q + 4; ++I) {
      const int lane = launder(lane_in);
      const int g = lane >> 4, c = lane & 15;
      if (I == Coop<NB>::col(q, wave)) {
#pragma unroll
        for (int r = 0; r < 4; ++r) {
          const int i = 16 * I + g + 4 * r;
          if (g + 4 * r == c && i < n) U[Coop<NB>::loc(I, q)][r] += shift;
        }
      }
    }
  }
}

template <int NB, int RHSMODE>
__device__ __forceinline__ double coop_factor(d4 (&U)[Coop<NB>::NT], double* rowbuf, double* Rbuf, double* Wbuf, double* scr,
                                              int wave, int lane_in, PivotAcc& pa, double* Lout, int ldl, int n,
                                              double* dvec = nullptr, double* Wout = nullptr, int ldw = 0,
                                              double* Lpack = nullptr, double* Wpack = nullptr, int kstop = NB) {
  using C = Coop<NB>;
  constexpr bool RHS = (RHSMODE == 1);
  double zq = 0.0;
#ifdef HGP_STAMPS
  unsigned long long cf_t = __builtin_readcyclecounter();
#define HGP_CF(i) do { unsigned long long n_ = __builtin_readcyclecounter(); pa.cf[i] += n_ - cf_t; cf_t = n_; } while (0)
#else
#define HGP_CF(i)
#endif
#pragma unroll
  for (int K = 0; K < NB; ++K) {
    if (K >= kstop) break;
    const int qK = K / 4, wK = C::owner(K);
    const int lane = launder(lane_in);
    const int g = lane >> 4, c = lane & 15;
    if (wave == wK) {
      double* Ld = (Lout != nullptr) ? Lout + (size_t)(16 * K) * ldl + 16 * K : nullptr;
      const d4 Wd = diag16_acc(U[C::loc(K, qK)], scr, lane, pa, 16 * K, Ld, ldl, n - 16 * K);
#pragma unroll
      for (int s = 0; s < 4; ++s) Wbuf[s * 64 + lane] = Wd[s];
      if (Wout != nullptr) {
#pragma unroll
        for (int s = 0; s < 4; ++s) {
          const int row = 16 * K + c, col = 16 * K + 4 * s + g;
          if (row < n && col < n) Wout[(size_t)row * ldw + col] = Wd[s];
        }
      }
      if (Wpack != nullptr) *reinterpret_cast<d4*>(Wpack + ((size_t)K * 64 + lane) * 4) = Wd;
      if (RHS) {
        const d4 rk = lds_tile_load(Rbuf, K, lane);
        d4 z = (d4){0.0, 0.0, 0.0, 0.0};
#pragma unroll
        for (int s = 0; s < 4; ++s) z = mfma(Wd[s], rk[s], z);
        lds_tile_store(Rbuf, K, lane, z);
      }
      if (RHSMODE == 2) {
        double p = 0.0;
#pragma unroll
        for (int s = 0; s < 4; ++s) p = fma(Wd[s], dvec[16 * K + 4 * s + g], p);
        p = xrow_sum(p);
        __builtin_amdgcn_wave_barrier();
        if (g == 0) {
          dvec[16 * K + c] = p;
          zq = fma(p, p, zq);
        }
      }
    }
    HGP_CF(0);
    __syncthreads();
    HGP_CF(1);
    d4 W;
#pragma unroll
    for (int s = 0; s < 4; ++s) W[s] = Wbuf[s * 64 + lane];
#pragma unroll
    for (int q = qK; q < C::NQ; ++q) {
      const int J = Coop<NB>::col(q, wave);
      if (J > K && J < NB) {
        const d4 t = U[C::loc(K, q)];
        d4 acc = (d4){0.0, 0.0, 0.0, 0.0};
#pragma unroll
        for (int s = 0; s < 4; ++s) acc = mfma(W[s], t[s], acc);
        U[C::loc(K, q)] = acc;
        lds_tile_store(rowbuf, J, lane, acc);
        if (Lout != nullptr) {
#pragma unroll
          for (int r = 0; r < 4; ++r) {
            const int row = 16 * J + c, col = 16 * K + g + 4 * r;
            if (row < n && col < n) Lout[(size_t)row * ldl + col] = acc[r];
          }
        }
        if (Lpack != nullptr) *reinterpret_cast<d4*>(Lpack + ((size_t)(J * (J - 1) / 2 + K) * 64 + lane) * 4) = acc;
      }
    }
    if (RHSMODE == 2) {
      double zr[4];
#pragma unroll
      for (int r = 0; r < 4; ++r) zr[r] = dvec[16 * K + g + 4 * r];
#pragma unroll
      for (int q = qK; q < C::NQ; ++q) {
        const int J = Coop<NB>::col(q, wave);
        if (J > K && J < NB) {
          double t = 0.0;
#pragma unroll
          for (int r = 0; r < 4; ++r) t = fma(U[C::loc(K, q)][r], zr[r], t);
          t = xrow_sum(t);
          if (g == 0) dvec[16 * J + c] -= t;
        }
      }
    }
    HGP_CF(2);
    __syncthreads();
    HGP_CF(3);
    if (K + 1 < NB) {
      d4 ucur = lds_tile_load(rowbuf, K + 1, lane);
#pragma unroll
      for (int I = K + 1; I < NB; ++I) {
        d4 unext = ucur;
        if (I + 1 < NB) unext = lds_tile_load(rowbuf, I + 1, lane);
#pragma unroll
        for (int q = I / 4; q < C::NQ; ++q) {
          if (C::col(q, wave) >= I) {
#pragma unroll
            for (int s = 0; s < 4; ++s) U[C::loc(I, q)] = mfma_sub(ucur[s], U[C::loc(K, q)][s], U[C::loc(I, q)]);
          }
        }
        ucur = unext;
      }
    }
    if (RHS) {
      const d4 zk = lds_tile_load(Rbuf, K, lane);
#pragma unroll
      for (int I = K + 1; I < NB; ++I) {
        if (C::owner(I) == wave) {
          const d4 uki = lds_tile_load(rowbuf, I, lane);
          d4 ri = lds_tile_load(Rbuf, I, lane);
#pragma unroll
          for (int s = 0; s < 4; ++s) ri = mfma_sub(uki[s], zk[s], ri);
          lds_tile_store(Rbuf, I, lane, ri);
        }
      }
    }
    HGP_CF(4);
  }
  __syncthreads();
  return zq;
}
#undef HGP_CF

__device__ __forceinline__ double coop_logdet_info(const PivotAcc& pa, int wave, int lane, double* red, int* redi, int& info) {
  if (lane == 0) {
    red[wave] = pa.logdet();
    redi[wave] = pa.info;
  }
  __syncthreads();
  const double ld = red[0] + red[1] + red[2] + red[3];
  int inf = 0;
#pragma unroll
  for (int w = 0; w < 4; ++w)
    if (redi[w] != 0 && (inf == 0 || redi[w] < inf)) inf = redi[w];
  info = inf;
  __syncthreads();
  return ld;
}

template <int NB_>
struct CoopH {
  static_assert(NB_ % 2 == 0 && NB_ <= 16, "CoopH: even NB <= 16");
  static constexpr int NB = NB_, NT = NB_ + 1, NW = NB_ / 2;
  __host__ __device__ static constexpr int slotA(int I) { return NB - I; }
  __host__ __device__ static constexpr int slotB(int I) { return I; }
  __host__ __device__ static constexpr int owner(int J) { return J < NW ? J : NB - 1 - J; }
  __host__ __device__ static constexpr int diag_slot(int K) { return K < NW ? slotA(K) : slotB(K); }
};

template <int NB>
__device__ __forceinline__ double cooph_diag_abs_mean(const d4 (&U)[CoopH<NB>::NT], int n, int wave, int lane_in, double shift,
                                                      double* red) {
  double s = 0.0;
#pragma unroll
  for (int K = 0; K < NB; ++K) {
    const int lane = launder(lane_in);
    const int g = lane >> 4, c = lane & 15;
    if (wave == CoopH<NB>::owner(K)) {
#pragma unroll
      for (int r = 0; r < 4; ++r) {
        const int i = 16 * K + g + 4 * r;
        if (g + 4 * r == c && i < n) s += fabs(U[CoopH<NB>::diag_slot(K)][r] + shift);
      }
    }
  }
  s = wave_sum(s);
  if (lane_in == 0) red[wave] = s;
  __syncthreads();
  double tot = 0.0;
#pragma unroll
  for (int w = 0; w < CoopH<NB>::NW; ++w) tot += red[w];
  __syncthreads();
  return tot / (double)n;
}

template <int NB>
__device__ __forceinline__ void cooph_add_diag(d4 (&U)[CoopH<NB>::NT], double shift, int n, int wave, int lane_in) {
#pragma unroll
  for (int K = 0; K < NB; ++K) {
    const int lane = launder(lane_in);
    const int g = lane >> 4, c = lane & 15;
    if (wave == CoopH<NB>::owner(K)) {
#pragma unroll
      for (int r = 0; r < 4; ++r) {
        const int i = 16 * K + g + 4 * r;
        if (g + 4 * r == c && i < n) U[CoopH<NB>::diag_slot(K)][r] += shift;
      }
    }
  }
}

template <int NB>
__device__ __forceinline__ void cooph_load_sym_upper(d4 (&U)[CoopH<NB>::NT], const double* __restrict__ A, int ld, int n, int wave,
                                                     int lane_in, double* scr_w) {
  using C = CoopH<NB>;
#pragma unroll
  for (int h = 0; h < 2; ++h) {
    const int lane = launder(lane_in);
    const int g = lane >> 4, c = lane & 15;
    const int J = h == 0 ? wave : NB - 1 - wave;
    d4 nat[NB], trn[NB];
#pragma unroll
    for (int I = 0; I < NB; ++I) {
      if (h == 0 && I >= C::NW) continue;
#pragma unroll
      for (int r = 0; r < 4; ++r) {
        const int i = 16 * I + g + 4 * r, j = 16 * J + c;
        nat[I][r] = (I <= J && i < n && j < n) ? A[(size_t)i * ld + j] : 0.0;
        const int i2 = 16 * J + g + 4 * r, j2 = 16 * I + c;
        trn[I][r] = (I < J && i2 < n && j2 < n) ? A[(size_t)i2 * ld + j2] : 0.0;
      }
    }
#pragma unroll
    for (int I = 0; I < NB; ++I) {
      if (h == 0 && I >= C::NW) continue;
      const d4 src = (I == J) ? nat[I] : trn[I];
#pragma unroll
      for (int r = 0; r < 4; ++r) scr_w[(g + 4 * r) * DIAG_LD + c] = src[r];
      __builtin_amdgcn_wave_barrier();
      d4 v = (d4){0.0, 0.0, 0.0, 0.0};
#pragma unroll
      for (int r = 0; r < 4; ++r) {
        const int i = 16 * I + g + 4 * r, j = 16 * J + c;
        const double t = scr_w[c * DIAG_LD + g + 4 * r];
        double x = 0.5 * (nat[I][r] + t);
        if (!(i < n && j < n)) x = (i == j) ? 1.0 : 0.0;
        if (I <= J) v[r] = x;
      }
      __builtin_amdgcn_wave_barrier();
      if (h == 0) U[C::slotA(I < C::NW ? I : 0)] = (I <= J) ? v : U[C::slotA(I < C::NW ? I : 0)];
      else if (I <= J) U[C::slotB(I)] = v;
    }
  }
}

template <int NB>
__device__ __forceinline__ double cooph_factor(d4 (&U)[CoopH<NB>::NT], double* rowbuf, double* Wbuf, double* scr, int wave,
                                               int lane_in, PivotAcc& pa, int n, double* dvec) {
  using C = CoopH<NB>;
  double zq = 0.0;
  const int JA = wave, JB = NB - 1 - wave;
#ifdef HGP_STAMPS
  unsigned long long cf_t = __builtin_readcyclecounter();
#define HGP_CF(i) do { unsigned long long n_ = __builtin_readcyclecounter(); pa.cf[i] += n_ - cf_t; cf_t = n_; } while (0)
#else
#define HGP_CF(i)
#endif
#pragma unroll
  for (int K = 0; K < NB; ++K) {
    const int lane = launder(lane_in);
    const int g = lane >> 4, c = lane & 15;
    if (wave == C::owner(K)) {
      const d4 Wd = diag16_acc(U[C::diag_slot(K)], scr, lane, pa, 16 * K, nullptr, 0, n - 16 * K);
#pragma unroll
      for (int s = 0; s < 4; ++s) Wbuf[s * 64 + lane] = Wd[s];
      double p = 0.0;
#pragma unroll
      for (int s = 0; s < 4; ++s) p = fma(Wd[s], dvec[16 * K + 4 * s + g], p);
      p = xrow_sum(p);
      __builtin_amdgcn_wave_barrier();
      if (g == 0) {
        dvec[16 * K + c] = p;
        zq = fma(p, p, zq);
      }
    }
    HGP_CF(0);
    __syncthreads();
    HGP_CF(1);
    d4 W;
#pragma unroll
    for (int s = 0; s < 4; ++s) W[s] = Wbuf[s * 64 + lane];
    double zr[4];
#pragma unroll
    for (int r = 0; r < 4; ++r) zr[r] = dvec[16 * K + g + 4 * r];
#pragma unroll
    for (int h = 0; h < 2; ++h) {
      if (h == 0 && K >= C::NW) continue;
      const int J = h == 0 ? JA : JB;
      const int sl = h == 0 ? C::slotA(K) : C::slotB(K);
      if (J > K) {
        const d4 t = U[sl];
        d4 acc = (d4){0.0, 0.0, 0.0, 0.0};
#pragma unroll
        for (int s = 0; s < 4; ++s) acc = mfma(W[s], t[s], acc);
        U[sl] = acc;
        lds_tile_store(rowbuf, J, lane, acc);
        double tq = 0.0;
#pragma unroll
        for (int r = 0; r < 4; ++r) tq = fma(acc[r], zr[r], tq);
        tq = xrow_sum(tq);
        if (g == 0) dvec[16 * J + c] -= tq;
      }
    }
    HGP_CF(2);
    __syncthreads();
    HGP_CF(3);
    if (K + 1 < NB) {
      d4 ucur = lds_tile_load(rowbuf, K + 1, lane);
#pragma unroll
      for (int I = K + 1; I < NB; ++I) {
        d4 unext = ucur;
        if (I + 1 < NB) unext = lds_tile_load(rowbuf, I + 1, lane);
        if (I < C::NW && K < C::NW && JA >= I) {
#pragma unroll
          for (int s = 0; s < 4; ++s) U[C::slotA(I)] = mfma_sub(ucur[s], U[C::slotA(K)][s], U[C::slotA(I)]);
        }
        if (JB >= I) {
#pragma unroll
          for (int s = 0; s < 4; ++s) U[C::slotB(I)] = mfma_sub(ucur[s], U[C::slotB(K)][s], U[C::slotB(I)]);
        }
        ucur = unext;
      }
    }
    HGP_CF(4);
  }
  __syncthreads();
  return zq;
}
#undef HGP_CF

constexpr int COOPH_SPIN_LIMIT = 1 << 22;

__device__ __forceinline__ void df_publish(int* p, int v, int lane) {
  __builtin_amdgcn_fence(__ATOMIC_RELEASE, "workgroup");
  if (lane == 0) __hip_atomic_store(p, v, __ATOMIC_RELAXED, __HIP_MEMORY_SCOPE_WORKGROUP);
#ifdef HGP_RACE_STRESS
  {
    const unsigned h = ((threadIdx.x >> 6) + 1u) * 2654435761u ^ (unsigned)(__builtin_readcyclecounter() >> 7);
    const unsigned n = __builtin_amdgcn_readfirstlane((h >> 5) & 7u);
    for (unsigned i = 0; i < n; ++i) __builtin_amdgcn_s_sleep(32);
  }
#endif
}
__device__ __forceinline__ void df_wait_ge(int* p, int v, int* err, bool hot = false) {
  int it = 0;
  while (__hip_atomic_load(p, __ATOMIC_RELAXED, __HIP_MEMORY_SCOPE_WORKGROUP) < v) {
    if (!hot) __builtin_amdgcn_s_sleep(1);
    if (++it > COOPH_SPIN_LIMIT) {
      *err = 1;
      break;
    }
  }
  __builtin_amdgcn_fence(__ATOMIC_ACQUIRE, "workgroup");
}
template <int NW>
__device__ __forceinline__ void df_wait_all_ge(int* tdone, int v, int lane, int* err) {
  int it = 0;
  while (!__all(__hip_atomic_load(&tdone[lane & (NW - 1)], __ATOMIC_RELAXED, __HIP_MEMORY_SCOPE_WORKGROUP) >= v)) {
    __builtin_amdgcn_s_sleep(1);
    if (++it > COOPH_SPIN_LIMIT) {
      *err = 1;
      break;
    }
  }
  __builtin_amdgcn_fence(__ATOMIC_ACQUIRE, "workgroup");
}

template <int NB, int RHS = 0>
__device__ __forceinline__ double cooph_factor_df(d4 (&U)[CoopH<NB>::NT], double* row0, double* row1, double* row2, double* Wall,
                                                  double* scr, int* flags, int wave, int lane_in, PivotAcc& pa, int n, double* dvec,
                                                  d4* RAp = nullptr, d4* RBp = nullptr, double* zbuf = nullptr,
                                                  double* Lpack = nullptr, double* Wpack = nullptr) {
  constexpr bool RP = (RHS == 1), NORHS = (RHS == 2);
  using C = CoopH<NB>;
  int* wdone = flags;
  int* tdone = flags + 1;
  int* err = flags + 9;
  int* rowpub = flags + 16;
  if (threadIdx.x < 16 + NB) flags[threadIdx.x] = 0;
  __syncthreads();
  double zq = 0.0;
  const int JA = wave, JB = NB - 1 - wave;
  double dpA = 0.0, dpB = 0.0;
#ifdef HGP_STAMPS
  unsigned long long cf_t = __builtin_readcyclecounter();
#define HGP_DF(i) do { unsigned long long n_ = __builtin_readcyclecounter(); pa.cf[i] += n_ - cf_t; cf_t = n_; } while (0)
#else
#define HGP_DF(i)
#endif

  auto do_diag = [&](auto Kc) {
    constexpr int K = decltype(Kc)::value;
    const int lane = launder(lane_in);
    const int g = lane >> 4, c = lane & 15;
    HGP_DF(4);
    __builtin_amdgcn_s_setprio(3);
    const d4 Wd = diag16_acc(U[C::diag_slot(K)], scr, lane, pa, 16 * K, nullptr, 0, n - 16 * K);
#pragma unroll
    for (int s = 0; s < 4; ++s) Wall[(K * 4 + s) * 64 + lane] = Wd[s];
    if (Wpack != nullptr) *reinterpret_cast<d4*>(Wpack + ((size_t)K * 64 + lane) * 4) = Wd;
    if constexpr (NORHS) {
    } else if constexpr (RP) {
      d4& rk = (K < C::NW) ? *RAp : *RBp;
      d4 z = (d4){0.0, 0.0, 0.0, 0.0};
#pragma unroll
      for (int s = 0; s < 4; ++s) z = mfma(Wd[s], rk[s], z);
      rk = z;
      lds_tile_store(zbuf, K, lane, z);
    } else {
      if constexpr (K > 0) {
        const double q = xrow_sum((K < C::NW) ? dpA : dpB);
        if (g == 0) dvec[16 * K + c] -= q;
        __builtin_amdgcn_wave_barrier();
      }
      double p = 0.0;
#pragma unroll
      for (int s = 0; s < 4; ++s) p = fma(Wd[s], dvec[16 * K + 4 * s + g], p);
      p = xrow_sum(p);
      __builtin_amdgcn_wave_barrier();
      if (g == 0) {
        dvec[16 * K + c] = p;
        zq = fma(p, p, zq);
      }
    }
    df_publish(wdone, K + 1, lane_in);
    __builtin_amdgcn_s_setprio(0);
    HGP_DF(0);
  };
  if (wave == C::owner(0)) do_diag(std::integral_constant<int, 0>{});
  static_for<0, NB>([&](auto Kc) {
    constexpr int K = decltype(Kc)::value;
    const int lane = launder(lane_in);
    const int g = lane >> 4, c = lane & 15;
    HGP_DF(4);
    df_wait_ge(wdone, K + 1, err, (K + 1 < NB) && wave == C::owner(K + 1 < NB ? K + 1 : 0));
    HGP_DF(1);
    d4 W;
#pragma unroll
    for (int s = 0; s < 4; ++s) W[s] = Wall[(K * 4 + s) * 64 + lane];
    double zr[4] = {0.0, 0.0, 0.0, 0.0};
    d4 zk = (d4){0.0, 0.0, 0.0, 0.0};
    if constexpr (NORHS) {
    } else if constexpr (RP) {
      zk = lds_tile_load(zbuf, K, lane);
    } else {
#pragma unroll
      for (int r = 0; r < 4; ++r) zr[r] = dvec[16 * K + g + 4 * r];
    }
    double* rb = (K % 3 == 0) ? row0 : (K % 3 == 1 ? row1 : row2);
    const bool haveA = (K < C::NW) && (JA > K), haveB = JB > K;
    if constexpr (K >= 3) {
      if (haveA || haveB) {
        if constexpr ((C::NW & (C::NW - 1)) == 0) df_wait_all_ge<C::NW>(tdone, K - 2, lane_in, err);
        else {
          for (int w = 0; w < C::NW; ++w) df_wait_ge(&tdone[w], K - 2, err);
        }
      }
    }
    HGP_DF(3);
    auto panel_col = [&](auto hc) -> d4 {
      constexpr int h = decltype(hc)::value;
      constexpr int sl = (h == 0) ? C::slotA(K < C::NW ? K : 0) : C::slotB(K);
      const int J = (h == 0) ? JA : JB;
      const d4 t = U[sl];
      d4 acc = (d4){0.0, 0.0, 0.0, 0.0};
#pragma unroll
      for (int s = 0; s < 4; ++s) acc = mfma(W[s], t[s], acc);
      U[sl] = acc;
      lds_tile_store(rb, J, lane, acc);
      if (Lpack != nullptr) *reinterpret_cast<d4*>(Lpack + ((size_t)(J * (J - 1) / 2 + K) * 64 + lane) * 4) = acc;
      if constexpr (NORHS) {
      } else if constexpr (RP) {
        d4& rj = (h == 0) ? *RAp : *RBp;
#pragma unroll
        for (int s = 0; s < 4; ++s) rj = mfma_sub(acc[s], zk[s], rj);
      } else {
#pragma unroll
        for (int r = 0; r < 4; ++r) {
          if (h == 0) dpA = fma(acc[r], zr[r], dpA);
          else dpB = fma(acc[r], zr[r], dpB);
        }
      }
      __builtin_amdgcn_fence(__ATOMIC_RELEASE, "workgroup");
      if (lane_in == 0) __hip_atomic_store(&rowpub[J], K + 1, __ATOMIC_RELAXED, __HIP_MEMORY_SCOPE_WORKGROUP);
      return acc;
    };
    constexpr int HC = (K + 1 < C::NW) ? 0 : 1;
    bool crit = false;
    if constexpr (K + 1 < NB) crit = (wave == C::owner(K + 1));
    if constexpr (K + 1 < NB) {
      if (crit) {
        const d4 acc = panel_col(std::integral_constant<int, HC>{});
        HGP_DF(2);
        constexpr int sd = C::diag_slot(K + 1);
#pragma unroll
        for (int s = 0; s < 4; ++s) U[sd] = mfma_sub(acc[s], acc[s], U[sd]);
        do_diag(std::integral_constant<int, K + 1>{});
      }
    }
    if (!(crit && HC == 0) && haveA) {
      if constexpr (K < C::NW) {
        panel_col(std::integral_constant<int, 0>{});
      }
    }
    if (!(crit && HC == 1) && haveB) {
      panel_col(std::integral_constant<int, 1>{});
    }
    HGP_DF(2);
    static_for<K + 1, NB>([&](auto Ic) {
      constexpr int I = decltype(Ic)::value;
      bool needA = (I < C::NW) && (K < C::NW) && (JA >= I), needB = JB >= I;
      if constexpr (I == K + 1) {
        if (crit && HC == 0) needA = false;
        if (crit && HC == 1) needB = false;
      }
      if (needA || needB) {
        HGP_DF(4);
        df_wait_ge(&rowpub[I], K + 1, err);
        HGP_DF(3);
        const d4 ucur = lds_tile_load(rb, I, lane);
        if constexpr (I < C::NW && K < C::NW) {
          if (needA) {
#pragma unroll
            for (int s = 0; s < 4; ++s) U[C::slotA(I)] = mfma_sub(ucur[s], U[C::slotA(K)][s], U[C::slotA(I)]);
          }
        }
        if (needB) {
#pragma unroll
          for (int s = 0; s < 4; ++s) U[C::slotB(I)] = mfma_sub(ucur[s], U[C::slotB(K)][s], U[C::slotB(I)]);
        }
      }
    });
    df_publish(&tdone[wave], K + 1, lane_in);
  });
  __syncthreads();
  if (*err) pa.info = 1;
  return zq;
}
#undef HGP_DF

template <int NB>
__device__ __forceinline__ double cooph_logdet_info(const PivotAcc& pa, int wave, int lane, double* red, int* redi, int& info) {
  if (lane == 0) {
    red[wave] = pa.logdet();
    redi[wave] = pa.info;
  }
  __syncthreads();
  double ld = 0.0;
  int inf = 0;
#pragma unroll
  for (int w = 0; w < CoopH<NB>::NW; ++w) {
    ld += red[w];
    if (redi[w] != 0 && (inf == 0 || redi[w] < inf)) inf = redi[w];
  }
  info = inf;
  __syncthreads();
  return ld;
}

}
```

Baseline: 15.42 million evals/s.

## Fuse kernel-matrix generation into inverse and acc-prep, collapse plan-update kernels

```diff
diff --git a/hdpgpc_amd/csrc/hgp_factor.hip b/hdpgpc_amd/csrc/hgp_factor.hip
--- a/hdpgpc_amd/csrc/hgp_factor.hip
+++ b/hdpgpc_amd/csrc/hgp_factor.hip
@@ -45,7 +45,24 @@
   }
 }
 
-template <int NB>
+__device__ __forceinline__ void gen_publish(const KtGenArgs& ga, int m, int TP, double c, double ell, double noise,
+                                            const SigmaDiagStats& ds, double jit, int tid, int nthreads) {
+  if (tid == 0) {
+    double* sc = ga.scal + 8 * m;
+    sc[0] = c;
+    sc[1] = ell;
+    sc[2] = noise;
+    sc[3] = ds.iso ? 1.0 : 0.0;
+    sc[4] = ds.mean;
+    sc[5] = jit;
+    sc[6] = 0.0;
+    if (m == 0 && ga.done) *ga.done = 0;
+  }
+  if (m == 0)
+    for (int i = tid; i < TP; i += nthreads) ga.xb_copy[i] = (i < ga.T) ? ga.xb[i] : 0.0;
+}
+
+template <int NB, bool GEN>
 __global__ __launch_bounds__(64 * WAVES) void k_wave_inv(PotrfArgs a) {
   __shared__ __attribute__((aligned(16))) double scr_all[WAVES * DIAG_SCR];
   const int wave = threadIdx.x >> 6, lane = threadIdx.x & 63;
@@ -55,12 +72,20 @@
   const int T = a.T;
   if (m >= a.b || 16 * Jc >= T) return;
   double* scr = scr_all + wave * DIAG_SCR;
-  const double* A = a.A + (size_t)m * T * T;
   d4 U[NB * (NB + 1) / 2];
   d4 R[NB];
-  if (a.symmetric) load_upper_only<NB>(U, A, T, T, lane);
-  else if constexpr (NB <= 6) load_sym_upper_burst<NB>(U, A, T, T, lane, scr);
-  else load_sym_upper<NB>(U, A, T, T, lane, scr);
+  if constexpr (GEN) {
+    const double cc = a.gen.theta[3 * m], ell = a.gen.theta[3 * m + 1];
+    const SigmaDiagStats ds = sigma_diag_stats(a.gen.Sigma + (size_t)m * a.gen.T * a.gen.T, a.gen.T, lane);
+    const double jit = 1e-4 * fmax(ds.mean_abs, F64_EPS);
+    if (Jc == 0) gen_publish(a.gen, m, T, cc, ell, a.gen.theta[3 * m + 2], ds, jit, lane, 64);
+    gen_kt_upper<NB>(U, a.gen.xb, cc, ell, jit, a.gen.T, lane);
+  } else {
+    const double* A = a.A + (size_t)m * T * T;
+    if (a.symmetric) load_upper_only<NB>(U, A, T, T, lane);
+    else if constexpr (NB <= 6) load_sym_upper_burst<NB>(U, A, T, T, lane, scr);
+    else load_sym_upper<NB>(U, A, T, T, lane, scr);
+  }
   {
     double sh = a.add;
     if (a.jitter_rel != 0.0) sh += a.jitter_rel * fmax(diag_abs_mean<NB>(U, T, lane, a.add), F64_EPS);
@@ -87,7 +112,9 @@
 template <int NB>
 void launch_wave_inv(const PotrfArgs& a, hipStream_t st) {
   const int waves = a.b * NB;
-  hipLaunchKernelGGL(k_wave_inv<NB>, dim3((waves + WAVES - 1) / WAVES), dim3(64 * WAVES), 0, st, a);
+  dispatch_bool(a.gen.xb != nullptr, [&](auto gen) {
+    hipLaunchKernelGGL((k_wave_inv<NB, decltype(gen)::value>), dim3((waves + WAVES - 1) / WAVES), dim3(64 * WAVES), 0, st, a);
+  });
 }
 
 struct ScoreArgs {
@@ -402,7 +429,7 @@
   }
 }
 
-template <int NB>
+template <int NB, bool GEN>
 __global__ __launch_bounds__(64 * WAVES) void k_coop_inv(PotrfArgs a) {
   using C = Coop<NB>;
   extern __shared__ __attribute__((aligned(16))) double smem[];
@@ -416,10 +443,18 @@
   const int m = blockIdx.x, Jc = blockIdx.y;
   const int T = a.T;
   if (16 * Jc >= T) return;
-  const double* A = a.A + (size_t)m * T * T;
   d4 U[C::NT];
-  coop_load_sym_upper<NB>(U, A, T, T, wave, lane, rowbuf + wave * DIAG_SCR);
-  __syncthreads();
+  if constexpr (GEN) {
+    const double cc = a.gen.theta[3 * m], ell = a.gen.theta[3 * m + 1];
+    const SigmaDiagStats ds = sigma_diag_stats(a.gen.Sigma + (size_t)m * a.gen.T * a.gen.T, a.gen.T, lane);
+    const double jit = 1e-4 * fmax(ds.mean_abs, F64_EPS);
+    if (Jc == 0) gen_publish(a.gen, m, T, cc, ell, a.gen.theta[3 * m + 2], ds, jit, (int)threadIdx.x, 64 * WAVES);
+    coop_gen_kt_upper<NB>(U, a.gen.xb, cc, ell, jit, a.gen.T, wave, lane);
+  } else {
+    const double* A = a.A + (size_t)m * T * T;
+    coop_load_sym_upper<NB>(U, A, T, T, wave, lane, rowbuf + wave * DIAG_SCR);
+    __syncthreads();
+  }
   {
     double sh = a.add;
     if (a.jitter_rel != 0.0) {
@@ -466,7 +501,6 @@
 int launch_coop_potrf(const PotrfArgs& a, hipStream_t st) {
   const size_t lds = sizeof(double) * Coop<NB>::LDS_DOUBLES;
   if (int rc_ = hgp_internal_ensure_dynamic_lds(reinterpret_cast<const void*>(&k_coop_potrf<NB>), lds)) return rc_;
-  if (int rc_ = hgp_internal_ensure_dynamic_lds(reinterpret_cast<const void*>(&k_coop_inv<NB>), lds)) return rc_;
   hipLaunchKernelGGL(k_coop_potrf<NB>, dim3(a.b), dim3(64 * WAVES), lds, st, a);
   if (a.Linv) {
     const int waves = a.b * NB;
@@ -479,9 +513,12 @@
 template <int NB>
 int launch_coop_inv_only(const PotrfArgs& a, hipStream_t st) {
   const size_t lds = sizeof(double) * Coop<NB>::LDS_DOUBLES;
-  if (int rc_ = hgp_internal_ensure_dynamic_lds(reinterpret_cast<const void*>(&k_coop_inv<NB>), lds)) return rc_;
-  hipLaunchKernelGGL(k_coop_inv<NB>, dim3(a.b, NB), dim3(64 * WAVES), lds, st, a);
-  return launch_status();
+  return dispatch_bool(a.gen.xb != nullptr, [&](auto gen) {
+    constexpr bool GEN = decltype(gen)::value;
+    if (int rc_ = hgp_internal_ensure_dynamic_lds(reinterpret_cast<const void*>(&k_coop_inv<NB, GEN>), lds)) return rc_;
+    hipLaunchKernelGGL((k_coop_inv<NB, GEN>), dim3(a.b, NB), dim3(64 * WAVES), lds, st, a);
+    return launch_status();
+  });
 }
 
 }
diff --git a/hdpgpc_amd/csrc/hgp_gemm.hip b/hdpgpc_amd/csrc/hgp_gemm.hip
--- a/hdpgpc_amd/csrc/hgp_gemm.hip
+++ b/hdpgpc_amd/csrc/hgp_gemm.hip
@@ -24,7 +24,8 @@
   const int row = 16 * ti + c, col = 16 * tj + c;
   int nk = (a.Kd + 3) / 4;
   if (a.triA && !a.tA) nk = min(nk, 4 * (ti + 1));
-  for (int k0 = 0; k0 < nk; k0 += TRIP) {
+  const int ks = a.ztz ? 4 * max(ti, tj) : 0;
+  for (int k0 = ks; k0 < nk; k0 += TRIP) {
     double av[TRIP], bv[TRIP];
 #pragma unroll
     for (int u = 0; u < TRIP; ++u) {
@@ -32,7 +33,9 @@
       av[u] = 0.0;
       bv[u] = 0.0;
       if (k < a.Kd) {
-        if (row < a.M) av[u] = a.tA ? A[(size_t)k * a.lda + row] : A[(size_t)row * a.lda + k];
+        if (a.symA) {
+          if (row < a.symA && k < a.symA) av[u] = 0.5 * (A[(size_t)row * a.lda + k] + A[(size_t)k * a.lda + row]);
+        } else if (row < a.M) av[u] = a.tA ? A[(size_t)k * a.lda + row] : A[(size_t)row * a.lda + k];
         if (col < a.N) bv[u] = a.tB ? B[(size_t)col * a.ldb + k] : B[(size_t)k * a.ldb + col];
       }
     }
@@ -155,7 +158,7 @@
     GemmArgs a = a0;
     a.boff = b0;
     const int nb = std::min(65535, batch - b0);
-    if (!a.tA && !a.tB && a.M % 32 == 0 && a.N % 32 == 0 && a.Kd % 32 == 0 && a.Kd > 128 &&
+    if (!a.tA && !a.tB && !a.symA && a.M % 32 == 0 && a.N % 32 == 0 && a.Kd % 32 == 0 && a.Kd > 128 &&
         (long)(a.M / 32) * (a.N / 32) * nb >= 2048) {
       const int nt2 = (a.M / 32) * (a.N / 32);
       hipLaunchKernelGGL(k_gemm22, dim3((nt2 + WAVES - 1) / WAVES, nb), dim3(64 * WAVES), 0, st, a);
diff --git a/hdpgpc_amd/csrc/hgp_internal.hpp b/hdpgpc_amd/csrc/hgp_internal.hpp
--- a/hdpgpc_amd/csrc/hgp_internal.hpp
+++ b/hdpgpc_amd/csrc/hgp_internal.hpp
@@ -55,8 +55,10 @@
   std::vector<int32_t> perm;
   std::vector<int> grp_beg, grp_end;
   std::vector<double> grp_ell;
-  double *d_theta, *d_scal, *d_A, *d_S, *d_Z, *d_Kinv, *d_P, *d_Q, *d_Mp, *d_ap, *d_xb;
+  double *d_theta, *d_scal, *d_A, *d_Z, *d_Kinv, *d_P, *d_Mp, *d_ap, *d_xb;
+  double* d_S = nullptr;
   int32_t* d_perm;
+  int32_t* d_done = nullptr;
   bool coop = false;
   double* d_escr = nullptr;
   int32_t* d_eflags = nullptr;
@@ -74,6 +76,16 @@
   int score_out = 0;
 };
 
+struct KtGenArgs {
+  const double* xb = nullptr;
+  const double* theta = nullptr;
+  const double* Sigma = nullptr;
+  int T = 0;
+  double* scal = nullptr;
+  double* xb_copy = nullptr;
+  int32_t* done = nullptr;
+};
+
 struct PotrfArgs {
   double* A;
   int T, b;
@@ -84,6 +96,7 @@
   int inv_info = 0;
   int symmetric = 0;
   double* Aout = nullptr;
+  KtGenArgs gen;
 };
 int hgp_internal_chol_inverse(const PotrfArgs& a, int NB, hipStream_t st);
 int hgp_internal_ensure_dynamic_lds(const void* fn, size_t bytes);
@@ -103,13 +116,15 @@
   long sD = 0;
   int boff = 0;
   int triA = 0;
+  int ztz = 0;
+  int symA = 0;
 };
 int hgp_internal_gemm(const GemmArgs& a, int batch, hipStream_t st);
 void hgp_internal_dot_batched(const double* X, const double* Y, long sX, long sY, long n, double scale, int accumulate, double* out, int b, hipStream_t st);
 void hgp_internal_colnorm_diag(const double* Z, const double* S, long sS, int T, double scale, int accumulate, double* out, int b, hipStream_t st);
 void hgp_internal_sub_batched(const double* A, const double* B, long sA, long sB, long n, double* C, int b, hipStream_t st);
 
-int hgp_internal_acc_prep(hgp_pairs_plan* p, const double* mean, hipStream_t st);
+int hgp_internal_acc_prep(hgp_pairs_plan* p, const double* mean, const double* Sigma, hipStream_t st);
 int hgp_internal_pairs_acc(const hgp_pairs_plan* p, const double* x, const double* y, int N, int Ts, const double* first_noise,
                            const int32_t* sel, double* out_quad, double* out_logdet, int32_t* out_info, hipStream_t st);
 size_t hgp_internal_acc_bytes(int TP, int K, size_t* sizes );
diff --git a/hdpgpc_amd/csrc/hgp_pairs_acc.hip b/hdpgpc_amd/csrc/hgp_pairs_acc.hip
--- a/hdpgpc_amd/csrc/hgp_pairs_acc.hip
+++ b/hdpgpc_amd/csrc/hgp_pairs_acc.hip
@@ -12,39 +12,12 @@
 __host__ __device__ constexpr int ntl(int NB) { return NB * (NB - 1) / 2; }
 __host__ __device__ constexpr int tl(int K, int Kp) { return K * (K - 1) / 2 + Kp; }
 
-__global__ void k_acc_flags(double* scal, int K, double tol, int32_t* acc_list) {
-  if (threadIdx.x != 0 || blockIdx.x != 0) return;
-  int n = 0;
-  for (int k = 0; k < K; ++k) {
-    const double ck = scal[8 * k] * scal[8 * k + 6];
-    const double bound = F64_EPS * ck * ck;
-    const bool flag = (tol == 0.0) || (tol > 0.0 && !(bound <= tol));
-    scal[8 * k + 7] = flag ? 1.0 : 0.0;
-    if (flag) acc_list[1 + n++] = k;
-  }
-  acc_list[0] = n;
-}
-
-template <int NB>
-__global__ __launch_bounds__(64) void k_acc_factor(double* A, int TP, const double* scal, int32_t* info) {
-  __shared__ __attribute__((aligned(16))) double scr[DIAG_SCR];
-  const int k = blockIdx.x, lane = threadIdx.x;
-  if (scal[8 * k + 7] == 0.0) return;
-  double* Ak = A + (size_t)k * TP * TP;
-  d4 U[NB * (NB + 1) / 2];
-  d4 R[NB];
-  load_upper_only<NB>(U, Ak, TP, TP, lane);
-  PivotAcc pa;
-  pa.init();
-  wave_factor<NB, 0>(U, R, scr, nullptr, nullptr, lane, pa, Ak, TP, TP);
-  if (lane == 0 && info && pa.info != 0) info[k] = pa.info;
-}
-
 struct AccPrepArgs {
-  const double* L;
-  const double* S;
+  double* L;
+  const double* Sigma;
   const double* mean;
   const double* scal;
+  const double* xb;
   int T, TP, NB;
   double* Lop;
   double* LTop;
@@ -53,14 +26,29 @@
   double* mu;
 };
 
+template <int NBF>
 __global__ __launch_bounds__(256) void k_acc_prep(AccPrepArgs a) {
   const int k = blockIdx.x;
   if (a.scal[8 * k + 7] == 0.0) return;
   const int lane = threadIdx.x & 63, g = lane >> 4, c = lane & 15;
   const int wv = blockIdx.y * 4 + (threadIdx.x >> 6), nwv = gridDim.y * 4;
-  const int NB = a.NB, TP = a.TP;
+  const int NB = a.NB, TP = a.TP, T = a.T;
+  if constexpr (NBF > 0) {
+    __shared__ __attribute__((aligned(16))) double scr[DIAG_SCR];
+    if (threadIdx.x < 64) {
+      const double* sc = a.scal + 8 * k;
+      d4 U[NBF * (NBF + 1) / 2];
+      d4 R[NBF];
+      gen_kt_upper<NBF>(U, a.xb, sc[0], sc[1], sc[5], T, lane);
+      PivotAcc pa;
+      pa.init();
+      wave_factor<NBF, 0>(U, R, scr, nullptr, nullptr, lane, pa, a.L + (size_t)k * TP * TP, TP, TP);
+    }
+    __threadfence();
+    __syncthreads();
+  }
   const double* L = a.L + (size_t)k * TP * TP;
-  const double* S = a.S + (size_t)k * TP * TP;
+  const double* Sg = a.Sigma + (size_t)k * T * T;
   const int nl = ntl(NB);
   double* Lop = a.Lop + (size_t)k * nl * 256;
   double* LTop = a.LTop + (size_t)k * nl * 256;
@@ -130,7 +118,10 @@
       const int t = it - nl - NB, Kb = t / NB, Kp = t % NB;
       d4 so;
 #pragma unroll
-      for (int s = 0; s < 4; ++s) so[s] = S[(size_t)(16 * Kp + 4 * s + g) * TP + 16 * Kb + c];
+      for (int s = 0; s < 4; ++s) {
+        const int i = 16 * Kp + 4 * s + g, j = 16 * Kb + c;
+        so[s] = (i < T && j < T) ? 0.5 * (Sg[(size_t)i * T + j] + Sg[(size_t)j * T + i]) : 0.0;
+      }
       *reinterpret_cast<d4*>(Sop + ((size_t)t * 64 + lane) * 4) = so;
     }
   }
@@ -407,16 +398,14 @@
   return tot;
 }
 
-int hgp_internal_acc_prep(hgp_pairs_plan* p, const double* mean, hipStream_t st) {
+int hgp_internal_acc_prep(hgp_pairs_plan* p, const double* mean, const double* Sigma, hipStream_t st) {
+  if (p->acc_tol < 0.0) return 0;
   const int K = p->K, TP = p->TP, NB = p->NB;
-  hipLaunchKernelGGL(k_acc_flags, dim3(1), dim3(64), 0, st, p->d_scal, K, p->acc_tol, p->d_acc_list);
-  if (p->acc_tol < 0.0) return launch_status();
+  AccPrepArgs a{p->d_A, Sigma, mean, p->d_scal, p->d_xb, p->T, TP, NB, p->d_Lop, p->d_LTop, p->d_Dop, p->d_Sop, p->d_mu};
   if (NB <= 8)
-    dispatch_nb_wave(TP, [&](auto nb) {
-      hipLaunchKernelGGL(k_acc_factor<decltype(nb)::value>, dim3(K), dim3(64), 0, st, p->d_A, TP, p->d_scal, (int32_t*)nullptr);
-    });
-  AccPrepArgs a{p->d_A, p->d_S, mean, p->d_scal, p->T, TP, NB, p->d_Lop, p->d_LTop, p->d_Dop, p->d_Sop, p->d_mu};
-  hipLaunchKernelGGL(k_acc_prep, dim3(K, 8), dim3(256), 0, st, a);
+    dispatch_nb_wave(TP, [&](auto nb) { hipLaunchKernelGGL(k_acc_prep<decltype(nb)::value>, dim3(K, 1), dim3(256), 0, st, a); });
+  else
+    hipLaunchKernelGGL(k_acc_prep<0>, dim3(K, 8), dim3(256), 0, st, a);
   return launch_status();
 }
 
diff --git a/hdpgpc_amd/csrc/hgp_plan.hip b/hdpgpc_amd/csrc/hgp_plan.hip
--- a/hdpgpc_amd/csrc/hgp_plan.hip
+++ b/hdpgpc_amd/csrc/hgp_plan.hip
@@ -18,6 +18,7 @@
   double* A;
   double* S;
   double* xb_copy;
+  int32_t* done;
 };
 
 __global__ __launch_bounds__(256) void k_prep_build(PrepArgs a) {
@@ -69,6 +70,7 @@
     sc[4] = mS;
     sc[5] = jit;
     sc[6] = 0.0;
+    if (k == 0) *a.done = 0;
   }
   if (k == 0 && blockIdx.y == 0)
     for (int i = tid; i < TP; i += 256) a.xb_copy[i] = (i < T) ? a.xb[i] : 0.0;
@@ -90,81 +92,152 @@
   }
 }
 
-struct PrepFinalArgs {
-  const double* Q;
+struct PlanFinalArgs {
   const double* Kinv;
+  const double* P;
   const double* mean;
   double* scal;
-  int T, TP;
+  int T, TP, K;
   double* Mp;
   double* ap;
   int interleave;
   int32_t* fb;
+  int32_t* done;
+  double tol;
+  int32_t* acc_list;
 };
 
-__global__ __launch_bounds__(256) void k_prep_final(PrepFinalArgs a) {
+__global__ __launch_bounds__(256) void k_plan_final(PlanFinalArgs a) {
+  __shared__ double tq[2][32][33], tk[2][32][33];
+  __shared__ double red[256];
   const int k = blockIdx.x, tid = threadIdx.x;
   if (a.fb && k == 0 && blockIdx.y == 0 && tid == 0) {
     a.fb[0] = 0;
     a.fb[1 + PAIRS_FB_CAP] = 0;
   }
   const int T = a.T, TP = a.TP;
+  const int nt = TP / 32, npair = nt * (nt + 1) / 2;
   const double c = a.scal[8 * k];
-  const double* Q = a.Q + (size_t)k * TP * TP;
   const double* Ki = a.Kinv + (size_t)k * TP * TP;
-  double* Mp = a.Mp + (size_t)k * TP * TP;
-  __shared__ double tq[32][33], tk[32][33];
-  const int NHh = (TP / 16) / 2, nt = TP / 32;
-  const int tx = tid & 31, ty = tid >> 5;
-  for (int t = blockIdx.y; t < nt * nt; t += gridDim.y) {
-    const int bi = t / nt, bj = t % nt;
+  const double* P = a.P + (size_t)k * TP * TP;
+  if ((int)blockIdx.y < npair) {
+    int bi = 0, t = blockIdx.y;
+    while (t >= nt - bi) {
+      t -= nt - bi;
+      ++bi;
+    }
+    const int bj = bi + t;
+    const int nh = (bi == bj) ? 1 : 2;
+    const int tx = tid & 31, ty = tid >> 5;
+    for (int h = 0; h < nh; ++h) {
+      const int I = h ? bj : bi, J = h ? bi : bj;
+#pragma unroll
+      for (int r = 0; r < 4; ++r) {
+        const int y = ty + 8 * r;
+        tk[h][y][tx] = Ki[(size_t)(32 * I + y) * TP + 32 * J + tx];
+      }
+    }
+    {
+      const int wave = tid >> 6, lane = tid & 63, g = lane >> 4, cc = lane & 15;
+      const int si = wave >> 1, sj = wave & 1;
+      const int nk = TP / 4;
+      constexpr int TRIP = 16;
+      const double* A0 = Ki + (size_t)(32 * bi + 16 * si + cc) * TP + g;
+      const double* B0 = P + (size_t)g * TP + 32 * bj + 16 * sj + cc;
+      const double* A1 = Ki + (size_t)(32 * bj + 16 * si + cc) * TP + g;
+      const double* B1 = P + (size_t)g * TP + 32 * bi + 16 * sj + cc;
+      d4 acc0 = (d4){0.0, 0.0, 0.0, 0.0}, acc1 = (d4){0.0, 0.0, 0.0, 0.0};
+      for (int k0 = 0; k0 < nk; k0 += TRIP) {
+        double av0[TRIP], bv0[TRIP], av1[TRIP], bv1[TRIP];
+#pragma unroll
+        for (int u = 0; u < TRIP; ++u) {
+          const bool in = k0 + u < nk;
+          const size_t kk = 4 * (size_t)(k0 + u);
+          av0[u] = in ? A0[kk] : 0.0;
+          bv0[u] = in ? B0[kk * TP] : 0.0;
+          av1[u] = (in && nh == 2) ? A1[kk] : 0.0;
+          bv1[u] = (in && nh == 2) ? B1[kk * TP] : 0.0;
+        }
+#pragma unroll
+        for (int u = 0; u < TRIP; ++u) {
+          acc0 = mfma(av0[u], bv0[u], acc0);
+          acc1 = mfma(av1[u], bv1[u], acc1);
+        }
+      }
+#pragma unroll
+      for (int r = 0; r < 4; ++r) {
+        tq[0][16 * si + g + 4 * r][16 * sj + cc] = acc0[r];
+        tq[1][16 * si + g + 4 * r][16 * sj + cc] = acc1[r];
+      }
+    }
     __syncthreads();
-#pragma unroll
-    for (int r = 0; r < 4; ++r) {
-      const int y = ty + 8 * r;
-      tq[y][tx] = Q[(size_t)(32 * bj + y) * TP + 32 * bi + tx];
-      tk[y][tx] = Ki[(size_t)(32 * bj + y) * TP + 32 * bi + tx];
-    }
+    double* Mp = a.Mp + (size_t)k * TP * TP;
+    const int NHh = (TP / 16) / 2;
+    for (int h = 0; h < nh; ++h) {
+      const int I = h ? bj : bi, J = h ? bi : bj, m = (nh == 2) ? 1 - h : 0;
+#pragma unroll
+      for (int r = 0; r < 4; ++r) {
+        const int y = ty + 8 * r;
+        const int i = 32 * I + y, j = 32 * J + tx;
+        double v = 0.0;
+        if (i < T && j < T) v = (c * c) * (0.5 * (tq[h][y][tx] + tq[m][tx][y]) - 0.5 * (tk[h][y][tx] + tk[m][tx][y]));
+        int jp = j;
+        if (a.interleave) {
+          const int hh = j / (16 * NHh), tl = (j / 16) % NHh, cc = j % 16;
+          const int loc = (tl < 2 * (NHh / 2)) ? 32 * (tl / 2) + 2 * cc + (tl & 1) : 16 * (NHh - 1) + cc;
+          jp = 16 * NHh * hh + loc;
+        }
+        Mp[(size_t)i * TP + jp] = v;
+      }
+    }
+  } else {
+    const double* mu = a.mean + (size_t)k * T;
+    const int i = ((int)blockIdx.y - npair) * 256 + tid;
+    double rs = 0.0;
+    if (i < TP) {
+      double s = 0.0;
+      if (i < T) {
+        for (int j0 = 0; j0 < T; j0 += 16) {
+          double kv[16];
+#pragma unroll
+          for (int u = 0; u < 16; ++u) kv[u] = (j0 + u < T) ? Ki[(size_t)(j0 + u) * TP + i] : 0.0;
+#pragma unroll
+          for (int u = 0; u < 16; ++u)
+            if (j0 + u < T) {
+              s = fma(kv[u], mu[j0 + u], s);
+              rs += fabs(kv[u]);
+            }
+        }
+      }
+      a.ap[(size_t)k * TP + i] = c * s;
+    }
+    red[tid] = rs;
     __syncthreads();
-#pragma unroll
-    for (int r = 0; r < 4; ++r) {
-      const int y = ty + 8 * r;
-      const int i = 32 * bi + y, j = 32 * bj + tx;
-      double v = 0.0;
-      if (i < T && j < T)
-        v = (c * c) * (0.5 * (Q[(size_t)i * TP + j] + tq[tx][y]) - 0.5 * (Ki[(size_t)i * TP + j] + tk[tx][y]));
-      int jp = j;
-      if (a.interleave) {
-        const int hh = j / (16 * NHh), tl = (j / 16) % NHh, cc = j % 16;
-        const int loc = (tl < 2 * (NHh / 2)) ? 32 * (tl / 2) + 2 * cc + (tl & 1) : 16 * (NHh - 1) + cc;
-        jp = 16 * NHh * hh + loc;
-      }
-      Mp[(size_t)i * TP + jp] = v;
-    }
-  }
-  const double* mu = a.mean + (size_t)k * T;
-  __shared__ double red[256];
-  double rmax = 0.0;
-  for (int i = blockIdx.y * 256 + tid; i < TP; i += gridDim.y * 256) {
-    double s = 0.0, rs = 0.0;
-    if (i < T) {
-#pragma unroll 8
-      for (int j = 0; j < T; ++j) {
-        const double kij = Ki[(size_t)j * TP + i];
-        s = fma(kij, mu[j], s);
-        rs += fabs(kij);
-      }
-    }
-    a.ap[(size_t)k * TP + i] = c * s;
-    rmax = fmax(rmax, rs);
-  }
-  red[tid] = rmax;
-  __syncthreads();
-  for (int o = 128; o > 0; o >>= 1) {
-    if (tid < o) red[tid] = fmax(red[tid], red[tid + o]);
-    __syncthreads();
-  }
-  if (tid == 0) atomicMax(reinterpret_cast<unsigned long long*>(a.scal + 8 * k + 6), (unsigned long long)__double_as_longlong(red[0]));
+    for (int o = 128; o > 0; o >>= 1) {
+      if (tid < o) red[tid] = fmax(red[tid], red[tid + o]);
+      __syncthreads();
+    }
+    if (tid == 0) atomicMax(reinterpret_cast<unsigned long long*>(a.scal + 8 * k + 6), (unsigned long long)__double_as_longlong(red[0]));
+  }
+  if (tid == 0) {
+    __threadfence();
+    const int nblocks = (int)(gridDim.x * gridDim.y);
+    if (atomicAdd(a.done, 1) == nblocks - 1) {
+      __threadfence();
+      int n = 0;
+      for (int kk = 0; kk < a.K; ++kk) {
+        const unsigned long long nb = __hip_atomic_load(reinterpret_cast<unsigned long long*>(a.scal + 8 * kk + 6), __ATOMIC_RELAXED,
+                                                        __HIP_MEMORY_SCOPE_AGENT);
+        const double ck = a.scal[8 * kk] * __longlong_as_double((long long)nb);
+        const double bound = F64_EPS * ck * ck;
+        const bool flag = (a.tol == 0.0) || (a.tol > 0.0 && !(bound <= a.tol));
+        a.scal[8 * kk + 7] = flag ? 1.0 : 0.0;
+        if (flag) a.acc_list[1 + n++] = kk;
+      }
+      a.acc_list[0] = n;
+      *a.done = 0;
+    }
+  }
 }
 
 static int tp_for(int n) {
@@ -185,12 +258,13 @@
   };
   take(p->d_theta, (size_t)K * 3 * sizeof(double));
   take(p->d_scal, (size_t)K * 8 * sizeof(double));
+  double* unused = nullptr;
   take(p->d_A, mat);
   take(p->d_S, mat);
   take(p->d_Z, mat);
   take(p->d_Kinv, mat);
   take(p->d_P, mat);
-  take(p->d_Q, mat);
+  take(unused, mat);
   take(p->d_Mp, mat);
   take(p->d_ap, (size_t)K * TP * sizeof(double));
   take(p->d_perm, (size_t)K * sizeof(int32_t));
@@ -213,7 +287,8 @@
   take(p->d_mu, sz[4]);
   take(p->d_sscr, sz[5]);
   take(p->d_acc_list, (size_t)(K + 1) * sizeof(int32_t));
-  take(p->d_fb, (size_t)(PAIRS_FB_CAP + 2) * sizeof(int32_t));
+  take(p->d_fb, (size_t)(PAIRS_FB_CAP + 3) * sizeof(int32_t));
+  if (base) p->d_done = p->d_fb + PAIRS_FB_CAP + 2;
   return o;
 }
 
@@ -257,7 +332,7 @@
     i = j;
   }
   plan_layout(p, T, Ts_max, K, (char*)dev_buf);
-  if (hipMemset(p->d_fb, 0, (size_t)(PAIRS_FB_CAP + 2) * sizeof(int32_t)) != hipSuccess) {
+  if (hipMemset(p->d_fb, 0, (size_t)(PAIRS_FB_CAP + 3) * sizeof(int32_t)) != hipSuccess) {
     delete p;
     return 1000 + (int)hipGetLastError();
   }
@@ -283,23 +358,40 @@
   if (!p || !x_basis || !mean || !Sigma) return -1;
   hipStream_t st = (hipStream_t)stream;
   const int K = p->K, T = p->T, TP = p->TP;
-  PrepArgs pa{x_basis, mean, Sigma, T, TP, K, p->d_theta, p->d_scal, p->d_A, p->d_S, p->d_xb};
-  hipLaunchKernelGGL(k_prep_build, dim3(K, 8), dim3(256), 0, st, pa);
   PotrfArgs fa{p->d_A, TP, K, 0.0, 0.0, p->d_Z, nullptr, info};
   fa.inv_info = 1;
   fa.symmetric = 1;
+  if (p->coop) {
+    PrepArgs pa{x_basis, mean, Sigma, T, TP, K, p->d_theta, p->d_scal, p->d_A, p->d_S, p->d_xb, p->d_done};
+    hipLaunchKernelGGL(k_prep_build, dim3(K, 8), dim3(256), 0, st, pa);
+  } else {
+    fa.gen.xb = x_basis;
+    fa.gen.theta = p->d_theta;
+    fa.gen.Sigma = Sigma;
+    fa.gen.T = T;
+    fa.gen.scal = p->d_scal;
+    fa.gen.xb_copy = p->d_xb;
+    fa.gen.done = p->d_done;
+  }
   if (int rc = hgp_internal_chol_inverse(fa, p->NB, st)) return rc;
   const long sm = (long)TP * TP;
   GemmArgs g1{p->d_Z, p->d_Z, p->d_Kinv, TP, TP, TP, TP, TP, TP, sm, sm, sm, 1.0, 0.0, 1, 0};
+  g1.ztz = 1;
   GemmArgs g2{p->d_S, p->d_Kinv, p->d_P, TP, TP, TP, TP, TP, TP, sm, sm, sm, 1.0, 0.0, 0, 0};
-  GemmArgs g3{p->d_Kinv, p->d_P, p->d_Q, TP, TP, TP, TP, TP, TP, sm, sm, sm, 1.0, 0.0, 0, 0};
+  if (!p->coop) {
+    g2.A = Sigma;
+    g2.lda = T;
+    g2.sA = (long)T * T;
+    g2.symA = T;
+  }
   hgp_internal_gemm(g1, K, st);
   hgp_internal_gemm(g2, K, st);
-  hgp_internal_gemm(g3, K, st);
-  PrepFinalArgs fin{p->d_Q, p->d_Kinv, mean, p->d_scal, T, TP, p->d_Mp, p->d_ap, p->coop ? 0 : 1, p->d_fb};
-  hipLaunchKernelGGL(k_prep_final, dim3(K, 8), dim3(256), 0, st, fin);
+  PlanFinalArgs fin{p->d_Kinv, p->d_P, mean, p->d_scal, T, TP, K, p->d_Mp, p->d_ap, p->coop ? 0 : 1, p->d_fb, p->d_done, p->acc_tol,
+                    p->d_acc_list};
+  const int nt = TP / 32;
+  hipLaunchKernelGGL(k_plan_final, dim3(K, nt * (nt + 1) / 2 + (TP + 255) / 256), dim3(256), 0, st, fin);
   if (p->d_eflags && p->nscr > 0 && hipMemsetAsync(p->d_eflags, 0, (p->nscr + 1) * sizeof(int32_t), st) != hipSuccess) return launch_status();
-  int rc = hgp_internal_acc_prep(p, mean, st);
+  int rc = hgp_internal_acc_prep(p, mean, Sigma, st);
   return rc ? rc : launch_status();
 }
 
diff --git a/hdpgpc_amd/csrc/tile_f64.hpp b/hdpgpc_amd/csrc/tile_f64.hpp
--- a/hdpgpc_amd/csrc/tile_f64.hpp
+++ b/hdpgpc_amd/csrc/tile_f64.hpp
@@ -1266,4 +1266,79 @@
   return ld;
 }
 
-}
+__device__ __forceinline__ double kt_entry(const double* __restrict__ xb, double c, double ell, double jit, int T, int i, int j) {
+  if (i < T && j < T) {
+    const double u = xb[i] / ell - xb[j] / ell;
+    double v = c * exp(-0.5 * (u * u));
+    if (i == j) v += jit;
+    return v;
+  }
+  return (i == j) ? 1.0 : 0.0;
+}
+
+template <int NB>
+__device__ __forceinline__ void gen_kt_upper(d4 (&U)[NB * (NB + 1) / 2], const double* __restrict__ xb, double c, double ell, double jit,
+                                             int T, int lane_in) {
+#pragma unroll
+  for (int I = 0; I < NB; ++I) {
+#pragma unroll
+    for (int J = I; J < NB; ++J) {
+      const int lane = launder(lane_in);
+      const int g = lane >> 4, cc = lane & 15;
+      d4 v;
+#pragma unroll
+      for (int r = 0; r < 4; ++r) v[r] = kt_entry(xb, c, ell, jit, T, 16 * I + g + 4 * r, 16 * J + cc);
+      U[tix(I, J, NB)] = v;
+    }
+  }
+}
+
+template <int NB>
+__device__ __forceinline__ void coop_gen_kt_upper(d4 (&U)[Coop<NB>::NT], const double* __restrict__ xb, double c, double ell, double jit,
+                                                  int T, int wave, int lane_in) {
+#pragma unroll
+  for (int q = 0; q < Coop<NB>::NQ; ++q) {
+    const int J = Coop<NB>::col(q, wave);
+#pragma unroll
+    for (int I = 0; I < 4 * q + 4; ++I) {
+      const int lane = launder(lane_in);
+      const int g = lane >> 4, cc = lane & 15;
+      d4 v = (d4){0.0, 0.0, 0.0, 0.0};
+      if (I <= J) {
+#pragma unroll
+        for (int r = 0; r < 4; ++r) v[r] = kt_entry(xb, c, ell, jit, T, 16 * I + g + 4 * r, 16 * J + cc);
+      }
+      U[Coop<NB>::loc(I, q)] = v;
+    }
+  }
+}
+
+struct SigmaDiagStats {
+  double mean_abs, mean;
+  int iso;
+};
+__device__ __forceinline__ double tree256_sum(double v0, double v1, double v2, double v3) {
+  double s = (v0 + v2) + (v1 + v3);
+#pragma unroll
+  for (int o = 32; o > 0; o >>= 1) s += __shfl_down(s, o, 64);
+  return __shfl(s, 0, 64);
+}
+__device__ __forceinline__ SigmaDiagStats sigma_diag_stats(const double* __restrict__ Sg, int T, int lane) {
+  double d[4];
+#pragma unroll
+  for (int q = 0; q < 4; ++q) {
+    const int i = lane + 64 * q;
+    d[q] = (i < T) ? Sg[(size_t)i * T + i] : 0.0;
+  }
+  SigmaDiagStats s;
+  s.mean_abs = tree256_sum(fabs(d[0]), fabs(d[1]), fabs(d[2]), fabs(d[3])) / T;
+  s.mean = tree256_sum(d[0], d[1], d[2], d[3]) / T;
+  int bad = 0;
+#pragma unroll
+  for (int q = 0; q < 4; ++q)
+    if (lane + 64 * q < T && !(fabs(d[q] - s.mean) <= 1e-8 + 1e-5 * fabs(s.mean))) bad = 1;
+  s.iso = __any(bad) ? 0 : 1;
+  return s;
+}
+
+}
```

New measurement: 15.51 million evals/s, median of 6. No clear change (+0.6%).
